# Sreyan88/audio-ssl

Hardware: AMD Instinct MI355X
Metric: upstream clips/sec (1s@16kHz, 64-mel) (higher is better)
Workload: dtype bf16; 1 GPU; delores-m upstream step (log-mel + 2 views + q/k conv encoders + MoCo + 3 Barlow heads + bwd + SGD), 1 s @ 16 kHz, 64 mel, batch 512/GPU, queue 65536; global_batch=512, parallelism=dp1

## Files before the change

audio-ssl_amd/csrc/bnpool.hip:

```cpp
#include "common.h"

namespace {

template <typename T_, bool SQ>
__global__ __launch_bounds__(256) void colstats_kernel(const T_* __restrict__ x, long M, int C, long ld, int rows_per_block,
                                                       double* __restrict__ sum, double* __restrict__ sumsq) {
    __shared__ float red[256][17];
    const int cg = threadIdx.x & 7, r0 = threadIdx.x >> 3;
    const int col0 = blockIdx.y * 64 + cg * 8;
    const long row_begin = (long)blockIdx.x * rows_per_block;
    const long row_end = min(M, row_begin + rows_per_block);
    x += (long)blockIdx.z * M * ld;
    sum += (long)blockIdx.z * C;
    if (SQ) sumsq += (long)blockIdx.z * C;
    float s[8], q[8];
#pragma unroll
    for (int i = 0; i < 8; ++i) { s[i] = 0.f; q[i] = 0.f; }
    if (col0 < C)
        for (long r = row_begin + r0; r < row_end; r += 32) {
            const Vec8<T_> v = Vec8<T_>::load(x + r * ld + col0);
#pragma unroll
            for (int i = 0; i < 8; ++i) { const float f = v.get(i); s[i] += f; if (SQ) q[i] += f * f; }
        }
#pragma unroll
// ... 369 lines not shown
    const int k8 = (int)(idx % 72);
    long pix = idx / 72;
    const int tap = k8 >> 3, c8 = k8 & 7;
    const int f = (int)(pix % Fi);
    const long r = pix / Fi;
    const int t = (int)(r % Ti);
    const long n = r / Ti;
    const int ff = f + tap / 3 - 1, tt = t + tap % 3 - 1;
    Vec8<T_> v = Vec8<T_>::zero();
    if (ff >= 0 && ff < Fi && tt >= 0 && tt < Ti) v = Vec8<T_>::load(X + (((n * Ti + tt) * Fi + ff) * 64 + c8 * 8));
    v.store(col + idx * 8);
}

template <typename T_>
__global__ void pack_conv_w_kernel(const float* __restrict__ W, T_* __restrict__ Wf, T_* __restrict__ Wd) {
    const int idx = blockIdx.x * 256 + threadIdx.x;
    if (idx >= 64 * 576) return;
    const int row = idx / 576, k = idx % 576, tap = k / 64, c = k % 64;
    Wf[idx] = from_f32<T_>(W[(row * 64 + c) * 9 + tap]);
    Wd[idx] = from_f32<T_>(W[(c * 64 + row) * 9 + (8 - tap)]);
}

template <typename T_>
__global__ void pack_conv_w2_kernel(const float* __restrict__ Wa, T_* __restrict__ Wfa, T_* __restrict__ Wda,
                                    const float* __restrict__ Wb, T_* __restrict__ Wfb, T_* __restrict__ Wdb) {
    const int idx = blockIdx.x * 256 + threadIdx.x;
    if (idx >= 64 * 576) return;
    const float* W = blockIdx.y ? Wb : Wa;
    T_* Wf = blockIdx.y ? Wfb : Wfa;
    T_* Wd = blockIdx.y ? Wdb : Wda;
    const int row = idx / 576, k = idx % 576, tap = k / 64, c = k % 64;
    Wf[idx] = from_f32<T_>(W[(row * 64 + c) * 9 + tap]);
    Wd[idx] = from_f32<T_>(W[(c * 64 + row) * 9 + (8 - tap)]);
}

__global__ void unpack_conv_dw_kernel(const float* __restrict__ dWp, float* __restrict__ dW) {
    const int idx = blockIdx.x * 256 + threadIdx.x;
    if (idx >= 64 * 576) return;
    const int co = idx / 576, k = idx % 576, tap = k / 64, ci = k % 64;
    dW[(co * 64 + ci) * 9 + tap] += dWp[idx];
}

}

#define DISPATCH_T(dtype, CALL_F32, CALL_BF16) do { if ((dtype) == 0) { CALL_F32; } else { CALL_BF16; } } while (0)

extern "C" int audiossl_colstats(int dtype, const void* x, int groups, long M, int C, long ld, int want_sq, double* sum,
                                 double* sumsq, void* stream) {
    ASSL_REQUIRE(x && sum && groups > 0 && M > 0 && C > 0 && (C % 8) == 0 && (ld % 8) == 0);
    ASSL_REQUIRE((dtype == 0 || dtype == 1) && (!want_sq || sumsq));
    hipStream_t s = static_cast<hipStream_t>(stream);
    const size_t nb = sizeof(double) * C * groups;
    if (want_sq && sumsq == sum + (size_t)C * groups) {
        ASSL_ZERO(sum, 2 * nb, s);
    } else {
        ASSL_ZERO(sum, nb, s);
        if (want_sq) ASSL_ZERO(sumsq, nb, s);
    }
    const int slabs = (C + 63) / 64;
    long it = (M * slabs * groups + 32L * 2048 - 1) / (32L * 2048);
    it = it < 1 ? 1 : (it > 128 ? 128 : it);
    const int rpb = 32 * (int)it;
    const dim3 grid(ceil_div(M, rpb), slabs, groups);
#define CS(TT, SQ) hipLaunchKernelGGL((colstats_kernel<TT, SQ>), grid, dim3(256), 0, s, static_cast<const TT*>(x), M, C, ld, rpb, sum, sumsq)
    if (dtype == 0) { if (want_sq) CS(float, true); else CS(float, false); }
    else            { if (want_sq) CS(bf16, true);  else CS(bf16, false); }
#undef CS
    ASSL_LAUNCH_CHECK();
}

extern "C" int audiossl_bn_finalize(const double* sum, const double* sumsq, int groups, double count, int C,
                                    const float* gamma, const float* beta, float* running_mean, float* running_var,
                                    float momentum, float eps, float* scale, float* shift, float* save_mean, float* save_rstd,
                                    void* stream) {
    ASSL_REQUIRE(sum && sumsq && scale && shift && save_mean && save_rstd && C > 0 && count > 0 && groups > 0);
    hipLaunchKernelGGL(bn_finalize_kernel, dim3(ceil_div(C, 256)), dim3(256), 0, static_cast<hipStream_t>(stream), sum, sumsq,
                       groups, count, C, gamma, beta, running_mean, running_var, momentum, eps, scale, shift, save_mean, save_rstd);
    ASSL_LAUNCH_CHECK();
}

extern "C" int audiossl_bn_relu_pool_fwd(int dtype, int ydtype, const void* Y, const float* scale, const float* shift, void* P,
                                         int N, int Ti, int Fi, void* stream) {
    ASSL_REQUIRE(Y && scale && shift && P && N > 0 && Ti >= 2 && Fi >= 2 && (Fi % 2) == 0 && (dtype == 0 || dtype == 1));
    ASSL_REQUIRE(ydtype == 0 || ydtype == dtype);
    const long total = (long)N * (Ti / 2) * (Fi / 2) * 8;
    hipStream_t s = static_cast<hipStream_t>(stream);
#define PF(TY, TO) hipLaunchKernelGGL((bn_relu_pool_fwd_kernel<TY, TO>), dim3(ceil_div(total, 256)), dim3(256), 0, s, \
        static_cast<const TY*>(Y), scale, shift, static_cast<TO*>(P), N, Ti, Fi)
    if (dtype == 0) PF(float, float); else if (ydtype == 0) PF(float, bf16); else PF(bf16, bf16);
#undef PF
    ASSL_LAUNCH_CHECK();
}

extern "C" int audiossl_bn_relu_pool_train_fwd(int dtype, int ydtype, const void* Y, const double* sum, const double* sumsq,
                                               int stat_replicas, double count,
                                               const float* gamma, const float* beta, float* running_mean, float* running_var,
                                               float momentum, float eps, void* P, float* scale, float* shift, float* save_mean,
                                               float* save_rstd, int N, int Ti, int Fi, void* stream) {
    ASSL_REQUIRE(Y && sum && sumsq && gamma && beta && P && scale && shift && save_mean && save_rstd && count > 0.0);
    ASSL_REQUIRE(stat_replicas >= 1 && (stat_replicas == 1 || sumsq == sum + 64));
    ASSL_REQUIRE(N > 0 && Ti >= 2 && Fi >= 2 && (Fi % 2) == 0 && (dtype == 0 || dtype == 1) && (ydtype == 0 || ydtype == dtype));
    const long total = (long)N * (Ti / 2) * (Fi / 2) * 8;
    hipStream_t s = static_cast<hipStream_t>(stream);
#define PF(TY, TO) hipLaunchKernelGGL((bn_relu_pool_train_fwd_kernel<TY, TO>), dim3(ceil_div(total, 256)), dim3(256), 0, s,          \
        static_cast<const TY*>(Y), sum, sumsq, stat_replicas, count, gamma, beta, running_mean, running_var, momentum, eps,      \
        static_cast<TO*>(P),                                                                                                      \
        scale, shift, save_mean, save_rstd, N, Ti, Fi)
    if (dtype == 0) PF(float, float); else if (ydtype == 0) PF(float, bf16); else PF(bf16, bf16);
#undef PF
    ASSL_LAUNCH_CHECK();
}

extern "C" int audiossl_tmean_fwd(int dtype, int out_f32, const void* P, void* xl, int N, int To, int Fo, void* stream) {
    ASSL_REQUIRE(P && xl && N > 0 && To > 0 && Fo > 0 && (dtype == 0 || dtype == 1));
    hipStream_t s = static_cast<hipStream_t>(stream);
#define TM(TI, TO_) hipLaunchKernelGGL((tmean_fwd_kernel<TI, TO_>), dim3(ceil_div(Fo * 8, 64), N), dim3(256), 0, s, \
        static_cast<const TI*>(P), static_cast<TO_*>(xl), N, To, Fo)
    if (dtype == 0) TM(float, float); else if (out_f32) TM(bf16, float); else TM(bf16, bf16);
#undef TM
    ASSL_LAUNCH_CHECK();
}

extern "C" int audiossl_tmean3_fwd(int dtype, int out_f32, const void* P1, void* x1, const float* x1_parts, int To1, int Fo1,
                                   const void* P2, void* x2, int To2, int Fo2, const void* P3, void* x3, int To3, int Fo3, int N,
                                   void* stream) {
    ASSL_REQUIRE(x1 && P2 && x2 && P3 && x3 && N > 0 && To1 > 0 && To2 > 0 && To3 > 0 && Fo1 > 0 && Fo2 > 0 && Fo3 > 0);
    ASSL_REQUIRE((P1 != nullptr) != (x1_parts != nullptr) && (!x1_parts || (out_f32 && dtype == 1)));
    ASSL_REQUIRE(dtype == 0 || dtype == 1);
    hipStream_t s = static_cast<hipStream_t>(stream);
    Tmean3 a{{P1, P2, P3}, {x1, x2, x3}, {To1, To2, To3}, {Fo1, Fo2, Fo3}, x1_parts};
    const int gx = ceil_div(max(Fo1, max(Fo2, Fo3)) * 8, 64);
#define TM3(TI, TO_) hipLaunchKernelGGL((tmean3_fwd_kernel<TI, TO_>), dim3(gx, N, 3), dim3(256), 0, s, a, N)
    if (dtype == 0) TM3(float, float); else if (out_f32) TM3(bf16, float); else TM3(bf16, bf16);
#undef TM3
    ASSL_LAUNCH_CHECK();
}

namespace {
__global__ void add_stat_kernel(const float* __restrict__ stat, float* dgamma, float* dbeta) {
    const int c = threadIdx.x;
    if (c < 64) { dbeta[c] += stat[c]; dgamma[c] += stat[64 + c]; }
}
}

static int bn_relu_pool_bwd_run(int phase, int dtype, int ydtype, int gdtype, const void* Y, const void* P, const void* dP, const void* dxl,
                                const float* scale, const float* shift, const float* mean, const float* rstd, float* stat,
                                const float* gstat, double count, void* dY, float* dgamma, float* dbeta, int N, int Ti, int Fi,
                                void* stream) {
    ASSL_REQUIRE(Y && dP && scale && shift && mean && rstd && stat);
    ASSL_REQUIRE(N > 0 && Ti >= 2 && Fi >= 2 && (Fi % 2) == 0 && (dtype == 0 || dtype == 1) && (gdtype == 0 || gdtype == dtype));
    ASSL_REQUIRE(ydtype == 0 || ydtype == dtype);
    ASSL_REQUIRE(phase == 1 || (dY && dgamma && dbeta));
    hipStream_t s = static_cast<hipStream_t>(stream);
    if (phase != 2) ASSL_ZERO(stat, sizeof(float) * 128 * 33, s);
    const long total = (long)N * ((Ti + 1) / 2) * (Fi / 2) * 8;
    const int grid = ceil_div(total, 256);
    const float inv_To = 1.f / (float)(Ti / 2);
    const float inv_count = (float)(1.0 / (phase == 2 ? count : (double)N * Ti * Fi));
    float* apply_stat = phase == 2 ? const_cast<float*>(gstat) : stat;
    const int fold = phase == 0;
#define BW(TY, AP, TG, TO, ST) hipLaunchKernelGGL((bn_relu_pool_bwd_kernel<TY, AP, TG, TO>), dim3(grid), dim3(256), 0, s,              \
        static_cast<const TY*>(Y), static_cast<const TG*>(dP), static_cast<const TG*>(dxl), inv_To, scale, shift, mean, rstd, ST, \
        inv_count, static_cast<TO*>(dY), N, Ti, Fi, (AP) ? fold : 0, dgamma, dbeta)
#define BWP(TG, TO) hipLaunchKernelGGL((bn_pool_bwd_stats_p_kernel<TO, TG>), dim3(pgrid), dim3(256), 0, s, static_cast<const TO*>(P),          \
        static_cast<const TG*>(dP), static_cast<const TG*>(dxl), inv_To, scale, shift, mean, rstd, stat, N, Ti / 2, Fi / 2)
#define BW2(TY, TG, TO) do { if (phase != 2) { if (P) BWP(TG, TO); else BW(TY, false, TG, TO, stat);                                       \
                                               if (!fold) hipLaunchKernelGGL(stat_reduce_kernel, dim3(1), dim3(128), 0, s, stat); }          \
                             if (phase != 1) BW(TY, true, TG, TO, apply_stat); } while (0)
    const long ptotal = (long)N * (Ti / 2) * (Fi / 2) * 8;
    const int pgrid = (int)min((long)2048, (ptotal + 255) / 256);
    if (dtype == 0) BW2(float, float, float);
    else if (ydtype == 0 && gdtype == 0) BW2(float, float, bf16);
    else if (ydtype == 0) BW2(float, bf16, bf16);
    else if (gdtype == 0) BW2(bf16, float, bf16);
    else BW2(bf16, bf16, bf16);
#undef BW2
#undef BWP
#undef BW
    if (phase == 2) hipLaunchKernelGGL(add_stat_kernel, dim3(1), dim3(64), 0, s, stat, dgamma, dbeta);
    ASSL_LAUNCH_CHECK();
}

extern "C" int audiossl_bn_relu_pool_bwd(int dtype, int ydtype, int gdtype, const void* Y, const void* dP, const void* dxl, const float* scale,
                                         const float* shift, const float* mean, const float* rstd, float* stat, void* dY,
                                         float* dgamma, float* dbeta, int N, int Ti, int Fi, void* stream) {
    return bn_relu_pool_bwd_run(0, dtype, ydtype, gdtype, Y, nullptr, dP, dxl, scale, shift, mean, rstd, stat, nullptr, 0.0, dY, dgamma, dbeta, N,
                                Ti, Fi, stream);
}
extern "C" int audiossl_bn_relu_pool_bwd_p(int dtype, int ydtype, int gdtype, const void* Y, const void* P, const void* dP, const void* dxl,
                                           const float* scale, const float* shift, const float* mean, const float* rstd, float* stat,
                                           void* dY, float* dgamma, float* dbeta, int N, int Ti, int Fi, void* stream) {
    ASSL_REQUIRE(P);
    return bn_relu_pool_bwd_run(0, dtype, ydtype, gdtype, Y, P, dP, dxl, scale, shift, mean, rstd, stat, nullptr, 0.0, dY, dgamma, dbeta, N,
                                Ti, Fi, stream);
}
extern "C" int audiossl_bn_relu_pool_bwd_stats(int dtype, int ydtype, int gdtype, const void* Y, const void* dP, const void* dxl,
                                               const float* scale, const float* shift, const float* mean, const float* rstd,
                                               float* stat, int N, int Ti, int Fi, void* stream) {
    return bn_relu_pool_bwd_run(1, dtype, ydtype, gdtype, Y, nullptr, dP, dxl, scale, shift, mean, rstd, stat, nullptr, 0.0, nullptr, nullptr,
                                nullptr, N, Ti, Fi, stream);
}
extern "C" int audiossl_bn_relu_pool_bwd_apply(int dtype, int ydtype, int gdtype, const void* Y, const void* dP, const void* dxl,
                                               const float* scale, const float* shift, const float* mean, const float* rstd,
                                               float* stat, const float* gstat, double count_global, void* dY, float* dgamma,
                                               float* dbeta, int N, int Ti, int Fi, void* stream) {
    ASSL_REQUIRE(gstat && count_global > 1.0);
    return bn_relu_pool_bwd_run(2, dtype, ydtype, gdtype, Y, nullptr, dP, dxl, scale, shift, mean, rstd, stat, gstat, count_global, dY, dgamma,
                                dbeta, N, Ti, Fi, stream);
}

extern "C" int audiossl_im2col3x3(int dtype, const void* X, void* col, int N, int Ti, int Fi, void* stream) {
    ASSL_REQUIRE(X && col && N > 0 && Ti > 0 && Fi > 0 && (dtype == 0 || dtype == 1));
    const long total = (long)N * Ti * Fi * 72;
    ASSL_REQUIRE((total + 255) / 256 < 2147483647L);
    hipStream_t s = static_cast<hipStream_t>(stream);
    DISPATCH_T(dtype,
        hipLaunchKernelGGL(im2col_kernel<float>, dim3(ceil_div(total, 256)), dim3(256), 0, s, static_cast<const float*>(X),
                           static_cast<float*>(col), N, Ti, Fi),
        hipLaunchKernelGGL(im2col_kernel<bf16>, dim3(ceil_div(total, 256)), dim3(256), 0, s, static_cast<const bf16*>(X),
                           static_cast<bf16*>(col), N, Ti, Fi));
    ASSL_LAUNCH_CHECK();
}

extern "C" int audiossl_pack_conv_w(int dtype, const float* W, void* Wf, void* Wd, void* stream) {
    ASSL_REQUIRE(W && Wf && Wd && (dtype == 0 || dtype == 1));
    hipStream_t s = static_cast<hipStream_t>(stream);
    DISPATCH_T(dtype,
        hipLaunchKernelGGL(pack_conv_w_kernel<float>, dim3(144), dim3(256), 0, s, W, static_cast<float*>(Wf), static_cast<float*>(Wd)),
        hipLaunchKernelGGL(pack_conv_w_kernel<bf16>, dim3(144), dim3(256), 0, s, W, static_cast<bf16*>(Wf), static_cast<bf16*>(Wd)));
    ASSL_LAUNCH_CHECK();
}

extern "C" int audiossl_pack_conv_w2(int dtype, const float* Wa, void* Wfa, void* Wda, const float* Wb, void* Wfb, void* Wdb, void* stream) {
    ASSL_REQUIRE(Wa && Wfa && Wda && Wb && Wfb && Wdb && (dtype == 0 || dtype == 1));
    hipStream_t s = static_cast<hipStream_t>(stream);
    DISPATCH_T(dtype,
        hipLaunchKernelGGL(pack_conv_w2_kernel<float>, dim3(144, 2), dim3(256), 0, s, Wa, static_cast<float*>(Wfa), static_cast<float*>(Wda),
                           Wb, static_cast<float*>(Wfb), static_cast<float*>(Wdb)),
        hipLaunchKernelGGL(pack_conv_w2_kernel<bf16>, dim3(144, 2), dim3(256), 0, s, Wa, static_cast<bf16*>(Wfa), static_cast<bf16*>(Wda),
                           Wb, static_cast<bf16*>(Wfb), static_cast<bf16*>(Wdb)));
    ASSL_LAUNCH_CHECK();
}

extern "C" int audiossl_unpack_conv_dw(const float* dWp, float* dW, void* stream) {
    ASSL_REQUIRE(dWp && dW);
    hipLaunchKernelGGL(unpack_conv_dw_kernel, dim3(144), dim3(256), 0, static_cast<hipStream_t>(stream), dWp, dW);
    ASSL_LAUNCH_CHECK();
}
```

audio-ssl_amd/csrc/conv.hip:

```cpp
#include <cstdlib>
#include "common.h"

namespace {

constexpr int CH = 64, KTOT = 576;
constexpr int WPITCH = KTOT + 8;
constexpr int PIXP = 72;
constexpr int PIXW = 96;

typedef __attribute__((address_space(3))) bf16x4* lds4_t;

struct ConvArgs {
    const bf16* X; const bf16* W; const float* bias; bf16* Y; double* sum; double* sumsq;
    int Ti, rows_total, tiles, out_f32, dbg, stat_rep;
};

template <int FI, int PITCH, int NTH = 256>
struct Halo {
    static constexpr int TT = 256 / FI;
    static constexpr int COLS = FI + 2;
    static constexpr int ELEMS = (TT + 2) * COLS * PITCH;
    static constexpr int NV = ((TT + 2) * FI * 8 + NTH - 1) / NTH;
    static constexpr int NVEC = (TT + 2) * FI * 8;
    Vec8<bf16> r[NV];
// ... 11 lines not shown
        for (int i = 0; i < NV; ++i) {
            const int v = threadIdx.x + i * NTH;
            const int row = v / (FI * 8), rem = v % (FI * 8);
            if (v < NVEC) r[i].store(lds + (row * COLS + (rem >> 3) + 1) * PITCH + (rem & 7) * 8);
        }
    }
    __device__ __forceinline__ static void zero_border(bf16* lds) {
        for (int i = threadIdx.x; i < (TT + 2) * 2 * 8; i += NTH) {
            const int row = i / 16, side = (i >> 3) & 1, c8 = i & 7;
            Vec8<bf16>::zero().store(lds + (row * COLS + side * (FI + 1)) * PITCH + c8 * 8);
        }
    }
};

template <int FI, int NW>
__global__ __launch_bounds__(64 * NW, 1) void conv3x3_kernel(ConvArgs a) {
    using H = Halo<FI, PIXP, 64 * NW>;
    constexpr int RT = 8 / NW;
    constexpr int TT = H::TT, COLS = H::COLS;
    extern __shared__ __attribute__((aligned(16))) char smem[];
    bf16* const wl = reinterpret_cast<bf16*>(smem);
    bf16* const hl = wl + CH * WPITCH;
    float* const red = reinterpret_cast<float*>(hl);

    const int lane = threadIdx.x & 63, wave = threadIdx.x >> 6;
    const int m = lane & 31, h = lane >> 5;
    for (int v = threadIdx.x; v < CH * KTOT / 8; v += 64 * NW) {
        const int row = v / (KTOT / 8), c = v % (KTOT / 8);
        Vec8<bf16>::load(a.W + row * KTOT + c * 8).store(wl + row * WPITCH + c * 8);
    }
    H::zero_border(hl);

    float ssum[2][16], ssq[2][16];
#pragma unroll
    for (int j = 0; j < 2; ++j)
#pragma unroll
        for (int r = 0; r < 16; ++r) { ssum[j][r] = 0.f; ssq[j][r] = 0.f; }
    f32x4 bias4[2][4];
#pragma unroll
    for (int j = 0; j < 2; ++j)
#pragma unroll
        for (int q = 0; q < 4; ++q)
            bias4[j][q] = a.bias ? *reinterpret_cast<const f32x4*>(a.bias + j * 32 + 8 * q + 4 * h) : f32x4{0.f, 0.f, 0.f, 0.f};
    H halo;
    int tile = blockIdx.x;
    if (tile < a.tiles) { halo.load(a.X, tile * TT, a.rows_total); halo.put(hl); }
    __syncthreads();

    for (; tile < a.tiles; tile += gridDim.x) {
        const int g0 = tile * TT;
        const int next = tile + gridDim.x;
        if (next < a.tiles && !(a.dbg & 2)) halo.load(a.X, next * TT, a.rows_total);

        int tl[RT], fcol[RT];
        bool ok[RT][3];
#pragma unroll
        for (int i = 0; i < RT; ++i) {
            const int rt = RT * wave + i;
            tl[i] = FI == 32 ? rt : 2 * rt + (m >> 4);
            fcol[i] = FI == 32 ? m : (m & 15);
            const int g = g0 + tl[i];
            const int ti = g % a.Ti;
#pragma unroll
            for (int dt = 0; dt < 3; ++dt) ok[i][dt] = g < a.rows_total && ti + dt - 1 >= 0 && ti + dt - 1 < a.Ti;
        }
        f32x16 acc[RT][2];
#pragma unroll
        for (int i = 0; i < RT; ++i)
#pragma unroll
            for (int j = 0; j < 2; ++j)
#pragma unroll
                for (int r = 0; r < 16; ++r) acc[i][j][r] = 0.f;

        if (!(a.dbg & 4))
#pragma unroll
        for (int tap = 0; tap < 9; ++tap) {
            const int dt = tap % 3, df = tap / 3;
#pragma unroll
            for (int cc = 0; cc < 4; ++cc) {
                Vec8<bf16> fa[RT], fb[2];
#pragma unroll
                for (int i = 0; i < RT; ++i) {
                    const bf16* p = hl + ((tl[i] + dt) * COLS + fcol[i] + df) * PIXP + cc * 16 + 8 * h;
                    fa[i] = ok[i][dt] ? Vec8<bf16>::load(p) : Vec8<bf16>::zero();
                }
#pragma unroll
                for (int j = 0; j < 2; ++j) fb[j] = Vec8<bf16>::load(wl + (j * 32 + m) * WPITCH + tap * 64 + cc * 16 + 8 * h);
#pragma unroll
                for (int i = 0; i < RT; ++i)
#pragma unroll
                    for (int j = 0; j < 2; ++j)
                        acc[i][j] = __builtin_amdgcn_mfma_f32_32x32x16_bf16(fb[j].v, fa[i].v, acc[i][j], 0, 0, 0);
            }
        }
#pragma unroll
        for (int i = 0; i < RT; ++i) {
            const int g = g0 + tl[i];
            if (g < a.rows_total && !(a.dbg & 1)) {
                const long o = ((long)g * FI + fcol[i]) * CH;
#pragma unroll
                for (int j = 0; j < 2; ++j)
#pragma unroll
                    for (int q = 0; q < 4; ++q) {
                        f32x4 v;
#pragma unroll
                        for (int e = 0; e < 4; ++e) {
                            v[e] = acc[i][j][4 * q + e] + bias4[j][q][e];
                            ssum[j][4 * q + e] += v[e];
                            ssq[j][4 * q + e] += v[e] * v[e];
                        }
                        const int co = j * 32 + 8 * q + 4 * h;
                        if (a.out_f32) *reinterpret_cast<f32x4*>(reinterpret_cast<float*>(a.Y) + o + co) = v;
                        else *reinterpret_cast<bf16x4*>(a.Y + o + co) = bf16x4{(bf16)v[0], (bf16)v[1], (bf16)v[2], (bf16)v[3]};
                    }
            }
        }
        __syncthreads();
        if (next < a.tiles) halo.put(hl);
        __syncthreads();
    }
    if (a.sum) {
#pragma unroll
        for (int j = 0; j < 2; ++j)
#pragma unroll
            for (int r = 0; r < 16; ++r) {
                float s = ssum[j][r], q = ssq[j][r];
#pragma unroll
                for (int o = 16; o > 0; o >>= 1) { s += __shfl_xor(s, o, 64); q += __shfl_xor(q, o, 64); }
                if (m == 0) {
                    const int co = j * 32 + (r & 3) + 8 * (r >> 2) + 4 * h;
                    red[(wave * 64 + co) * 2] = s; red[(wave * 64 + co) * 2 + 1] = q;
                }
            }
        __syncthreads();
        if (threadIdx.x < 128) {
            const int c = threadIdx.x >> 1, k = threadIdx.x & 1;
            double t = 0.0;
#pragma unroll
            for (int w = 0; w < NW; ++w) t += (double)red[(w * 64 + c) * 2 + k];
            const int rep = (blockIdx.x % a.stat_rep) * 128;
            atomicAdd(k == 0 ? &a.sum[rep + c] : &a.sumsq[rep + c], t);
        }
    }
}

template <int FI>
struct WsGeom {
    static constexpr int TT = 256 / FI, COLS = FI + 2, ROWS = TT + 2, SEGS = FI / 8;
    static constexpr int UNITS = ROWS * SEGS;
    static constexpr int UPW = (UNITS + 3) / 4;
    static constexpr int BYTES = ROWS * COLS * 128;
};

template <int FI, bool STATS, bool F32OUT, int PF = 2>
__global__ __launch_bounds__(256, 1) void conv3x3_ws_kernel(ConvArgs a) {
    using G = WsGeom<FI>;
    constexpr int TT = G::TT, COLS = G::COLS;
    typedef __attribute__((address_space(3))) void* lptr_t;
    extern __shared__ __attribute__((aligned(16))) char smem[];
    float* const biasl = reinterpret_cast<float*>(smem + 2 * G::BYTES);
    float* const red = biasl + 64;
    constexpr int OPIX = F32OUT ? 256 : 128;
    char* const stg = reinterpret_cast<char*>(red + 4 * 64 * 2) + (threadIdx.x >> 6) * 64 * OPIX;
    char* const zblk = reinterpret_cast<char*>(red + 4 * 64 * 2) + 4 * 64 * OPIX;
    if (threadIdx.x < 32) *reinterpret_cast<f32x4*>(zblk + threadIdx.x * 16) = f32x4{0.f, 0.f, 0.f, 0.f};

    const int lane = threadIdx.x & 63, wave = __builtin_amdgcn_readfirstlane(threadIdx.x >> 6);
    const int m = lane & 31, h = lane >> 5;
    long* const rts = (!STATS && (a.dbg & 16) && threadIdx.x == 0 && (blockIdx.x == 0 || blockIdx.x == gridDim.x - 1))
                          ? reinterpret_cast<long*>(a.sum) + 64 + (blockIdx.x ? 8 : 0) : nullptr;
    if (rts) rts[0] = __builtin_amdgcn_s_memrealtime();

    {
        bf16* const wl = reinterpret_cast<bf16*>(smem);
        Vec8<bf16> tmp[CH * KTOT / 8 / 256];
#pragma unroll
        for (int k = 0; k < CH * KTOT / 8 / 256; ++k) tmp[k] = Vec8<bf16>::load(a.W + (threadIdx.x + 256 * k) * 8);
#pragma unroll
        for (int k = 0; k < CH * KTOT / 8 / 256; ++k) {
            const int v = threadIdx.x + 256 * k, row = v / (KTOT / 8), c = v % (KTOT / 8);
            tmp[k].store(wl + row * WPITCH + c * 8);
        }
        __syncthreads();
    }
    Vec8<bf16> wr[2][36];
#pragma unroll
    for (int j = 0; j < 2; ++j)
#pragma unroll
        for (int ks = 0; ks < 36; ++ks)
            wr[j][ks] = Vec8<bf16>::load(reinterpret_cast<const bf16*>(smem) + (j * 32 + m) * WPITCH + ks * 16 + 8 * h);
#pragma unroll
    for (int ks = 0; ks < 36; ++ks) {
        asm volatile("" : "+v"(wr[0][ks].v));
        asm volatile("" : "+a"(wr[1][ks].v));
    }

    __syncthreads();
    for (int i = threadIdx.x; i < 2 * G::ROWS * 2 * 8; i += 256) {
        const int b = i / (G::ROWS * 16), r = (i / 16) % G::ROWS, side = (i >> 3) & 1, c8 = i & 7;
        *reinterpret_cast<f32x4*>(smem + b * G::BYTES + (r * COLS + side * (FI + 1)) * 128 + c8 * 16) = f32x4{0.f, 0.f, 0.f, 0.f};
    }
    if (threadIdx.x < 64) biasl[threadIdx.x] = a.bias ? a.bias[threadIdx.x] : 0.f;

    if (rts) { asm volatile("s_waitcnt vmcnt(0)" ::: "memory"); rts[3] = __builtin_amdgcn_s_memrealtime(); }
    const __amdgpu_buffer_rsrc_t rsrc = __builtin_amdgcn_make_buffer_rsrc(const_cast<bf16*>(a.X), 0, (unsigned)((long)a.rows_total * FI * 128), 0x00020000);
    const int pl = lane >> 3, cp = lane & 7;
    const int key0 = ((1 + pl) >> 1) & 7;
    const int voff0 = pl * 128 + ((cp ^ key0) << 4), voff1 = pl * 128 + ((cp ^ key0 ^ 4) << 4);
    auto dma_unit = [&](int g0, char* buf, int i) {
        {
            const int u = wave + 4 * i;
            if (u < G::UNITS) {
                const int row = u / G::SEGS, seg = u % G::SEGS;
                const int gr = g0 - 1 + row;
                const int so = (gr >= 0 && gr < a.rows_total) ? (gr * FI + 8 * seg) * 128 : 0x7FFFFF00;
                __builtin_amdgcn_raw_ptr_buffer_load_lds(rsrc, (lptr_t)(buf + (row * COLS + 1 + 8 * seg) * 128), 16, (seg & 1) ? voff1 : voff0, so, 0, 0);
            }
        }
    };
    auto dma_tile = [&](int g0, char* buf) {
#pragma unroll
        for (int i = 0; i < G::UPW; ++i) dma_unit(g0, buf, i);
    };

    int tl[2];
    const int fcol = FI == 32 ? m : (m & 15);
#pragma unroll
    for (int i = 0; i < 2; ++i) {
        const int rt = 2 * wave + i;
        tl[i] = FI == 32 ? rt : 2 * rt + (m >> 4);
    }
    int hs[3];
#pragma unroll
    for (int df = 0; df < 3; ++df) hs[df] = (h ^ (((fcol + df) >> 1) & 7)) << 4;

    constexpr int NS = F32OUT ? 4 : 8;
    float ssum[NS], ssq[NS];
    if (STATS) {
#pragma unroll
        for (int e = 0; e < NS; ++e) { ssum[e] = 0.f; ssq[e] = 0.f; }
    }

    int tile = blockIdx.x, cur = 0;
    if (tile < a.tiles) dma_tile(tile * TT, smem);
    asm volatile("s_waitcnt vmcnt(0) lgkmcnt(0)" ::: "memory");
    __builtin_amdgcn_s_barrier();

    long* const ts = (!STATS && (a.dbg & 16) && blockIdx.x == 0 && threadIdx.x == 0) ? reinterpret_cast<long*>(a.sum) : nullptr;
    int tsi = 0;
    if (rts) rts[1] = __builtin_amdgcn_s_memrealtime();
    for (; tile < a.tiles; tile += gridDim.x, cur ^= 1) {
        if (ts) ts[tsi++] = __builtin_amdgcn_s_memtime();
        const int g0 = tile * TT;
        const int next = tile + gridDim.x;
        if (next < a.tiles && !(a.dbg & 2)) dma_tile(next * TT, smem + (cur ^ 1) * G::BYTES);
        const char* const hl = smem + cur * G::BYTES;

        int bdt[2][3];
#pragma unroll
        for (int i = 0; i < 2; ++i) {
            const int g = g0 + tl[i];
            const int ti = g % a.Ti;
#pragma unroll
            for (int dt = 0; dt < 3; ++dt) {
                const bool ok = g < a.rows_total && ti + dt - 1 >= 0 && ti + dt - 1 < a.Ti;
                bdt[i][dt] = ok ? (int)(size_t)((lptr_t)const_cast<char*>(hl)) + ((tl[i] + dt) * COLS + fcol) * 128
                                : (int)(size_t)((lptr_t)zblk);
            }
        }
        f32x16 acc[2][2];
#pragma unroll
        for (int j = 0; j < 2; ++j)
#pragma unroll
            for (int q = 0; q < 4; ++q) {
                const f32x4 b4 = *reinterpret_cast<const f32x4*>(biasl + j * 32 + 8 * q + 4 * h);
#pragma unroll
                for (int e = 0; e < 4; ++e) { acc[0][j][4 * q + e] = b4[e]; acc[1][j][4 * q + e] = b4[e]; }
            }

        Vec8<bf16> fa[PF + 1][2];
        auto fetch = [&](int ks, Vec8<bf16> (&f)[2]) {
            const int tap = ks >> 2, cc = ks & 3, dt = tap % 3, df = tap / 3;
#pragma unroll
            for (int i = 0; i < 2; ++i)
                f[i] = Vec8<bf16>::load(reinterpret_cast<const bf16*>((const char*)(lptr_t)(size_t)(bdt[i][dt] + df * 128 + (hs[df] ^ (cc * 32)))));
        };
        if (!(a.dbg & 4)) {
#pragma unroll
        for (int ks = 0; ks < PF; ++ks) fetch(ks, fa[ks]);
#pragma unroll
        for (int ks = 0; ks < 36; ++ks) {
            if (ks + PF < 36) fetch(ks + PF, fa[(ks + PF) % (PF + 1)]);
            __builtin_amdgcn_sched_barrier(0);
            Vec8<bf16> (&f)[2] = fa[ks % (PF + 1)];
#pragma unroll
            for (int i = 0; i < 2; ++i) {
#pragma unroll
                for (int j = 0; j < 2; ++j)
                    acc[i][j] = __builtin_amdgcn_mfma_f32_32x32x16_bf16(wr[j][ks].v, f[i].v, acc[i][j], 0, 0, 0);
            }
            __builtin_amdgcn_sched_barrier(0);
        }
        }
        if (ts) ts[tsi++] = __builtin_amdgcn_s_memtime();
        asm volatile("s_waitcnt vmcnt(0)" ::: "memory");
        if (ts) ts[tsi++] = __builtin_amdgcn_s_memtime();
        if (!(a.dbg & 1)) {
#pragma unroll
            for (int i = 0; i < 2; ++i) {
                char* const st = stg + i * 32 * OPIX;
#pragma unroll
                for (int j = 0; j < 2; ++j)
#pragma unroll
                    for (int q = 0; q < 4; ++q) {
                        const int slot = j * 8 + 2 * q + h;
                        const f32x4 v = f32x4{acc[i][j][4 * q], acc[i][j][4 * q + 1], acc[i][j][4 * q + 2], acc[i][j][4 * q + 3]};
                        if (F32OUT) *reinterpret_cast<f32x4*>(st + m * 256 + ((slot ^ (m & 15)) << 4)) = v;
                        else *reinterpret_cast<bf16x4*>(st + m * 128 + ((slot ^ ((m >> 1) & 15)) << 3)) =
                                 bf16x4{(bf16)v[0], (bf16)v[1], (bf16)v[2], (bf16)v[3]};
                    }
            }
            asm volatile("s_waitcnt lgkmcnt(0)" ::: "memory");
#pragma unroll
            for (int i = 0; i < 2; ++i) {
                const char* const st = stg + i * 32 * OPIX;
                const int grow = g0 + (2 * wave + i) * (32 / FI);
                const int prow_ok = a.rows_total - grow;
                char* const yrow = reinterpret_cast<char*>(a.Y) + (long)grow * FI * 64 * (F32OUT ? 4 : 2);
                if (F32OUT) {
#pragma unroll
                    for (int it = 0; it < 8; ++it) {
                        const int p = it * 4 + (lane >> 4), c = lane & 15;
                        const f32x4 v = *reinterpret_cast<const f32x4*>(st + p * 256 + ((c ^ (p & 15)) << 4));
                        if ((p >> (FI == 32 ? 5 : 4)) < prow_ok) {
                            *reinterpret_cast<f32x4*>(yrow + p * 256 + c * 16) = v;
                            if (STATS) {
#pragma unroll
                                for (int e = 0; e < 4; ++e) { ssum[e] += v[e]; ssq[e] += v[e] * v[e]; }
                            }
                        }
                    }
                } else {
#pragma unroll
                    for (int it = 0; it < 4; ++it) {
                        const int p = it * 8 + (lane >> 3), c = lane & 7, k = (p >> 1) & 15;
                        f32x4 v = *reinterpret_cast<const f32x4*>(st + p * 128 + ((c ^ (k >> 1)) << 4));
                        if (k & 1) v = f32x4{v[2], v[3], v[0], v[1]};
                        if ((p >> (FI == 32 ? 5 : 4)) < prow_ok) {
                            *reinterpret_cast<f32x4*>(yrow + p * 128 + c * 16) = v;
                            if (STATS) {
                                const bf16x8 hv = __builtin_bit_cast(bf16x8, v);
#pragma unroll
                                for (int e = 0; e < 8; ++e) {
                                    const float x = (float)hv[e];
                                    ssum[e] += x; ssq[e] += x * x;
                                }
                            }
                        }
                    }
                }
            }
        }
        if (ts) ts[tsi++] = __builtin_amdgcn_s_memtime();
        asm volatile("s_waitcnt lgkmcnt(0)" ::: "memory");
        __builtin_amdgcn_s_barrier();
    }
    if (rts) rts[2] = __builtin_amdgcn_s_memrealtime();
    if (STATS) {
#pragma unroll
        for (int e = 0; e < NS; ++e) {
            float s = ssum[e], q = ssq[e];
#pragma unroll
            for (int o = 64 / NS; o < 64; o <<= 1) { s += __shfl_xor(s, o, 64); q += __shfl_xor(q, o, 64); }
            if (lane < 64 / NS) {
                const int co = lane * NS + e;
                red[(wave * 64 + co) * 2] = s; red[(wave * 64 + co) * 2 + 1] = q;
            }
        }
        __syncthreads();
        if (threadIdx.x < 128) {
            const int c = threadIdx.x >> 1, k = threadIdx.x & 1;
            double t = 0.0;
#pragma unroll
            for (int w = 0; w < 4; ++w) t += (double)red[(w * 64 + c) * 2 + k];
            const int rep = (blockIdx.x % a.stat_rep) * 128;
            atomicAdd(k == 0 ? &a.sum[rep + c] : &a.sumsq[rep + c], t);
        }
    }
}

__host__ __device__ __forceinline__ int wg_cot(int w, int n) { return n < 8 ? (n & 1) : (w & 1); }
__host__ __device__ __forceinline__ int wg_nt(int w, int n) { return n < 8 ? 4 * w + (n >> 1) : 16 + (w >> 1); }

struct WgradArgs {
    const bf16* dY; const bf16* X; float* dW; int Ti, rows_total, tiles;
    float* partial;
    int dbg;
};

template <int FI, int KG>
__global__ __launch_bounds__(256 * KG, 1) void conv3x3_wgrad_kernel(WgradArgs a) {
    using H = Halo<FI, PIXW, 256 * KG>;
    constexpr int TT = H::TT, COLS = H::COLS;
    constexpr int NTH = 256 * KG;
    constexpr int NVY = 256 * 8 / NTH;
    extern __shared__ __attribute__((aligned(16))) char smem[];
    bf16* const yl = reinterpret_cast<bf16*>(smem);
    bf16* const hl = yl + 256 * PIXW;

    const int lane = threadIdx.x & 63, wave = (threadIdx.x >> 6) & 3, grp = threadIdx.x >> 8;
    const int h = lane >> 5, half = (lane >> 4) & 1, q = (lane & 15) >> 2, p = lane & 3;
    H::zero_border(hl);

    f32x16 acc[9];
#pragma unroll
    for (int n = 0; n < 9; ++n)
#pragma unroll
        for (int r = 0; r < 16; ++r) acc[n][r] = 0.f;

    H halo;
    Vec8<bf16> ry[NVY];
    auto load_y = [&](int g0) {
#pragma unroll
        for (int i = 0; i < NVY; ++i) {
            const int v = threadIdx.x + i * NTH;
            const long pix = (long)g0 * FI + (v >> 3);
            ry[i] = pix < (long)a.rows_total * FI ? Vec8<bf16>::load(a.dY + pix * CH + (v & 7) * 8) : Vec8<bf16>::zero();
        }
    };
    auto put_y = [&]() {
#pragma unroll
        for (int i = 0; i < NVY; ++i) {
            const int v = threadIdx.x + i * NTH;
            ry[i].store(yl + (v >> 3) * PIXW + (v & 7) * 8);
        }
    };
    int tile = blockIdx.x;
    if (tile < a.tiles) { halo.load(a.X, tile * TT, a.rows_total); load_y(tile * TT); halo.put(hl); put_y(); }
    __syncthreads();

    for (; tile < a.tiles; tile += gridDim.x) {
        const int g0 = tile * TT;
        const int next = tile + gridDim.x;
        if (next < a.tiles && !(a.dbg & 2)) { halo.load(a.X, next * TT, a.rows_total); load_y(next * TT); }

#pragma unroll 1
        for (int ks = grp * (16 / KG); ks < (grp + 1) * (16 / KG) && !(a.dbg & 4); ++ks) {
            const int t_local = FI == 32 ? (ks >> 1) : ks;
            const int f0 = FI == 32 ? (ks & 1) * 16 : 0;
            const int g = g0 + t_local;
            if (g >= a.rows_total) break;
            const int ti = g % a.Ti;
            const bool okt[3] = {ti - 1 >= 0, true, ti + 1 < a.Ti};
            bf16x8 fa[2];
#pragma unroll
            for (int c2 = 0; c2 < 2; ++c2) {
                const bf16* ay = yl + (ks * 16 + 8 * h + q) * PIXW + c2 * 32 + 16 * half + 4 * p;
                const bf16x4 a0 = __builtin_amdgcn_ds_read_tr16_b64_v4bf16((lds4_t)ay);
                const bf16x4 a1 = __builtin_amdgcn_ds_read_tr16_b64_v4bf16((lds4_t)(ay + 4 * PIXW));
                fa[c2] = bf16x8{a0[0], a0[1], a0[2], a0[3], a1[0], a1[1], a1[2], a1[3]};
            }
            bf16x8 fb;
#pragma unroll
            for (int n = 0; n < 9; ++n) {
                if (n == 8 || (n & 1) == 0) {
                    const int nt = wg_nt(wave, n), tap = nt >> 1, cih = nt & 1;
                    const int dt = tap % 3, df = tap / 3;
                    const bf16* bx = hl + ((t_local + dt) * COLS + f0 + df + 8 * h + q) * PIXW + cih * 32 + 16 * half + 4 * p;
                    const bf16x4 b0 = __builtin_amdgcn_ds_read_tr16_b64_v4bf16((lds4_t)bx);
                    const bf16x4 b1 = __builtin_amdgcn_ds_read_tr16_b64_v4bf16((lds4_t)(bx + 4 * PIXW));
                    const bf16 z = (bf16)0.f;
                    fb = okt[dt] ? bf16x8{b0[0], b0[1], b0[2], b0[3], b1[0], b1[1], b1[2], b1[3]} : bf16x8{z, z, z, z, z, z, z, z};
                }
                const int c2 = wg_cot(wave, n);
                acc[n] = __builtin_amdgcn_mfma_f32_32x32x16_bf16(c2 ? fa[1] : fa[0], fb, acc[n], 0, 0, 0);
            }
        }
        __syncthreads();
        if (next < a.tiles) { halo.put(hl); put_y(); }
        __syncthreads();
    }
    if (a.partial) {
        if (KG == 2) {
            f32x4* xch = reinterpret_cast<f32x4*>(smem);
            __syncthreads();
            if (grp == 1) {
#pragma unroll
                for (int n = 0; n < 9; ++n)
#pragma unroll
                    for (int r4 = 0; r4 < 4; ++r4)
                        xch[((wave * 9 + n) * 4 + r4) * 64 + lane] = f32x4{acc[n][4 * r4], acc[n][4 * r4 + 1], acc[n][4 * r4 + 2], acc[n][4 * r4 + 3]};
            }
            __syncthreads();
            if (grp == 1) return;
            f32x4* part = reinterpret_cast<f32x4*>(a.partial + (long)blockIdx.x * (CH * KTOT));
#pragma unroll
            for (int n = 0; n < 9; ++n)
#pragma unroll
                for (int r4 = 0; r4 < 4; ++r4) {
                    const f32x4 o = xch[((wave * 9 + n) * 4 + r4) * 64 + lane];
                    part[((wave * 9 + n) * 4 + r4) * 64 + lane] = f32x4{acc[n][4 * r4] + o[0], acc[n][4 * r4 + 1] + o[1], acc[n][4 * r4 + 2] + o[2], acc[n][4 * r4 + 3] + o[3]};
                }
            return;
        }
        f32x4* part = reinterpret_cast<f32x4*>(a.partial + (long)blockIdx.x * (CH * KTOT));
#pragma unroll
        for (int n = 0; n < 9; ++n)
#pragma unroll
            for (int r4 = 0; r4 < 4; ++r4)
                part[((wave * 9 + n) * 4 + r4) * 64 + lane] = f32x4{acc[n][4 * r4], acc[n][4 * r4 + 1], acc[n][4 * r4 + 2], acc[n][4 * r4 + 3]};
        return;
    }
#pragma unroll
    for (int n = 0; n < 9; ++n) {
        const int nt = wg_nt(wave, n), tap = nt >> 1, cih = nt & 1;
        const int col = tap * 64 + cih * 32 + (lane & 31);
#pragma unroll
        for (int r = 0; r < 16; ++r) {
            const int co = wg_cot(wave, n) * 32 + (r & 3) + 8 * (r >> 2) + 4 * h;
            atomicAdd(&a.dW[co * KTOT + col], acc[n][r]);
        }
    }
}

__global__ __launch_bounds__(256) void wgrad_reduce_kernel(const float* __restrict__ partial, int nparts, float* __restrict__ dW) {
    const int i = blockIdx.x * 256 + threadIdx.x;
    if (i >= CH * KTOT) return;
    float s0 = 0.f, s1 = 0.f, s2 = 0.f, s3 = 0.f;
    int w = blockIdx.y;
    const int step = gridDim.y;
    for (; w + 3 * step < nparts; w += 4 * step) {
        s0 += partial[(long)w * (CH * KTOT) + i];
        s1 += partial[(long)(w + step) * (CH * KTOT) + i];
        s2 += partial[(long)(w + 2 * step) * (CH * KTOT) + i];
        s3 += partial[(long)(w + 3 * step) * (CH * KTOT) + i];
    }
    for (; w < nparts; w += step) s0 += partial[(long)w * (CH * KTOT) + i];
    const int e = i & 3, lane = (i >> 2) & 63, r4 = (i >> 8) & 3, wn = i >> 10;
    const int wave = wn / 9, n = wn - wave * 9;
    const int nt = wg_nt(wave, n), tap = nt >> 1, cih = nt & 1;
    const int col = tap * 64 + cih * 32 + (lane & 31);
    const int co = wg_cot(wave, n) * 32 + e + 8 * r4 + 4 * (lane >> 5);
    atomicAdd(&dW[co * KTOT + col], (s0 + s1) + (s2 + s3));
}

template <typename K>
int set_lds(K kernel, size_t bytes) {
    return hipFuncSetAttribute(reinterpret_cast<const void*>(kernel), hipFuncAttributeMaxDynamicSharedMemorySize, (int)bytes) ==
           hipSuccess ? 0 : -1;
}

}

extern "C" int audiossl_conv3x3_fwd(const void* X, const void* W, const float* bias, void* Y, int out_f32, double* sum,
                                    double* sumsq, int stat_replicas, int N, int Ti, int Fi, void* stream) {
    ASSL_REQUIRE(X && W && Y && N > 0 && Ti > 0 && (Fi == 32 || Fi == 16) && (!sum == !sumsq));
    ASSL_REQUIRE(stat_replicas >= 1 && stat_replicas <= 64 && (stat_replicas == 1 || !sum || sumsq == sum + 64));
    if (!ASSL_ALIGNED16(X) || !ASSL_ALIGNED16(W) || !ASSL_ALIGNED16(Y)) return ASSL_EALIGN;
    hipStream_t s = static_cast<hipStream_t>(stream);
#ifdef AUDIOSSL_ABLATE
    static const int conv_dbg = getenv("AUDIOSSL_CONV_DBG") ? atoi(getenv("AUDIOSSL_CONV_DBG")) : 0;
#else
    constexpr int conv_dbg = 0;
#endif
    if (sum && !(conv_dbg & 16)) {
        if (sumsq == sum + 64) {
            ASSL_ZERO(sum, sizeof(double) * 128 * stat_replicas, s);
        } else {
            ASSL_ZERO(sum, sizeof(double) * 64, s);
            ASSL_ZERO(sumsq, sizeof(double) * 64, s);
        }
    }
    const int rows = N * Ti, TT = 256 / Fi, tiles = (rows + TT - 1) / TT;
    ConvArgs a{static_cast<const bf16*>(X), static_cast<const bf16*>(W), bias, static_cast<bf16*>(Y), sum, sumsq, Ti, rows, tiles, out_f32, conv_dbg, stat_replicas};
    const int grid = tiles < 256 ? tiles : 256;
    static const int ws = getenv("AUDIOSSL_CONV_WS") ? atoi(getenv("AUDIOSSL_CONV_WS")) : 1;
    if (ws && (long)rows * Fi * 128 < 0x7FFFFF00L) {
        static bool wattr[8] = {false, false, false, false, false, false, false, false};
#define WS_LAUNCH(FI_, ST_, F32_, SLOT)                                                                    \
    do {                                                                                                  \
        const size_t lds = 2 * WsGeom<FI_>::BYTES + sizeof(float) * (64 + 4 * 64 * 2) + 4 * 64 * (F32_ ? 256 : 128) + 512; \
        if (!wattr[SLOT]) { if (set_lds(conv3x3_ws_kernel<FI_, ST_, F32_>, lds)) return ASSL_ELAUNCH; wattr[SLOT] = true; } \
        hipLaunchKernelGGL((conv3x3_ws_kernel<FI_, ST_, F32_>), dim3(grid), dim3(256), lds, s, a);       \
    } while (0)
        if (Fi == 32) {
            if (sum && !(conv_dbg & 16)) { if (out_f32) WS_LAUNCH(32, true, true, 0); else WS_LAUNCH(32, true, false, 1); }
            else     { if (out_f32) WS_LAUNCH(32, false, true, 2); else WS_LAUNCH(32, false, false, 3); }
        } else {
            if (sum) { if (out_f32) WS_LAUNCH(16, true, true, 4); else WS_LAUNCH(16, true, false, 5); }
            else     { if (out_f32) WS_LAUNCH(16, false, true, 6); else WS_LAUNCH(16, false, false, 7); }
        }
#undef WS_LAUNCH
        ASSL_LAUNCH_CHECK();
    }
    static const int nw = getenv("AUDIOSSL_CONV_WAVES") ? atoi(getenv("AUDIOSSL_CONV_WAVES")) : 8;
    static bool attr[4] = {false, false, false, false};
#define CONV_LAUNCH(FI_, NW_, SLOT)                                                                       \
    do {                                                                                                  \
        const size_t lds = sizeof(bf16) * (CH * WPITCH + Halo<FI_, PIXP>::ELEMS);                         \
        if (!attr[SLOT]) { if (set_lds(conv3x3_kernel<FI_, NW_>, lds)) return ASSL_ELAUNCH; attr[SLOT] = true; } \
        hipLaunchKernelGGL((conv3x3_kernel<FI_, NW_>), dim3(grid), dim3(64 * NW_), lds, s, a);           \
    } while (0)
    if (Fi == 32) { if (nw == 8) CONV_LAUNCH(32, 8, 0); else CONV_LAUNCH(32, 4, 1); }
    else          { if (nw == 8) CONV_LAUNCH(16, 8, 2); else CONV_LAUNCH(16, 4, 3); }
#undef CONV_LAUNCH
    ASSL_LAUNCH_CHECK();
}

extern "C" int audiossl_conv3x3_wgrad(const void* dY, const void* X, float* dWp, float* workspace, long workspace_floats, int N,
                                      int Ti, int Fi, void* stream) {
    ASSL_REQUIRE(dY && X && dWp && N > 0 && Ti > 0 && (Fi == 32 || Fi == 16));
    if (!ASSL_ALIGNED16(X) || !ASSL_ALIGNED16(dY)) return ASSL_EALIGN;
    hipStream_t s = static_cast<hipStream_t>(stream);
    const int rows = N * Ti, TT = 256 / Fi, tiles = (rows + TT - 1) / TT;
    const int grid = tiles < 256 ? tiles : 256;
    const bool two_stage = workspace != nullptr && workspace_floats >= (long)grid * CH * KTOT;
#ifdef AUDIOSSL_ABLATE
    static const int wg_dbg = getenv("AUDIOSSL_CONV_DBG") ? atoi(getenv("AUDIOSSL_CONV_DBG")) : 0;
#else
    constexpr int wg_dbg = 0;
#endif
    WgradArgs a{static_cast<const bf16*>(dY), static_cast<const bf16*>(X), dWp, Ti, rows, tiles, two_stage ? workspace : nullptr, wg_dbg};
    static const int kg_env = getenv("AUDIOSSL_WGRAD_KG") ? atoi(getenv("AUDIOSSL_WGRAD_KG")) : 0;
    const int kg = kg_env ? kg_env : (two_stage ? 2 : 1);
    static bool attr[4] = {false, false, false, false};
#define WGRAD_LAUNCH(FI_, KG_, SLOT)                                                                      \
    do {                                                                                                  \
        const size_t lds = max(sizeof(bf16) * (256 * PIXW + Halo<FI_, PIXW>::ELEMS), (size_t)(KG_ == 2 ? 4 * 9 * 16 * 64 * 4 : 0)); \
        if (!attr[SLOT]) { if (set_lds(conv3x3_wgrad_kernel<FI_, KG_>, lds)) return ASSL_ELAUNCH; attr[SLOT] = true; } \
        hipLaunchKernelGGL((conv3x3_wgrad_kernel<FI_, KG_>), dim3(grid), dim3(256 * KG_), lds, s, a);    \
    } while (0)
    if (Fi == 32) { if (kg == 2) WGRAD_LAUNCH(32, 2, 0); else WGRAD_LAUNCH(32, 1, 1); }
    else          { if (kg == 2) WGRAD_LAUNCH(16, 2, 2); else WGRAD_LAUNCH(16, 1, 3); }
#undef WGRAD_LAUNCH
    if (two_stage)
        hipLaunchKernelGGL(wgrad_reduce_kernel, dim3(CH * KTOT / 256, 8), dim3(256), 0, s, workspace, grid, dWp);
    ASSL_LAUNCH_CHECK();
}
```

audio-ssl_amd/csrc/heads.hip:

```cpp
#include "common.h"

namespace {

template <typename T_, typename TO>
__global__ __launch_bounds__(256) void maxmean_fwd_kernel(const T_* __restrict__ H, TO* __restrict__ y, uint8_t* __restrict__ arg,
                                                          int N, int Tt, int D) {
    const long idx = (long)blockIdx.x * 256 + threadIdx.x;
    const int D8 = D / 8;
    if (idx >= (long)N * D8) return;
    const int d8 = (int)(idx % D8);
    const long n = idx / D8;
    float mx[8], sm[8];
    int am[8];
    for (int t = 0; t < Tt; ++t) {
        const Vec8<T_> v = Vec8<T_>::load(H + ((n * Tt + t) * D + d8 * 8));
#pragma unroll
        for (int i = 0; i < 8; ++i) {
            const float f = v.get(i);
            if (t == 0) { mx[i] = f; sm[i] = f; am[i] = 0; }
            else { sm[i] += f; if (f > mx[i]) { mx[i] = f; am[i] = t; } }
        }
    }
    Vec8<TO> o;
    const float inv = 1.f / (float)Tt;
#pragma unroll
    for (int i = 0; i < 8; ++i) { o.set(i, mx[i] + sm[i] * inv); arg[n * D + d8 * 8 + i] = (uint8_t)am[i]; }
    o.store(y + n * D + d8 * 8);
}

template <typename T_, typename TG>
__global__ __launch_bounds__(256) void maxmean_bwd_kernel(const TG* __restrict__ dy, const uint8_t* __restrict__ arg,
                                                          const T_* __restrict__ H, T_* __restrict__ dA, int N, int Tt, int D) {
    const long idx = (long)blockIdx.x * 256 + threadIdx.x;
    const int D8 = D / 8;
    if (idx >= (long)N * Tt * D8) return;
    const int d8 = (int)(idx % D8);
    const long r = idx / D8;
    const int t = (int)(r % Tt);
    const long n = r / Tt;
    const Vec8<TG> g = Vec8<TG>::load(dy + n * D + d8 * 8);
    const Vec8<T_> h = Vec8<T_>::load(H + idx * 8);
    Vec8<T_> o;
    const float inv = 1.f / (float)Tt;
#pragma unroll
    for (int i = 0; i < 8; ++i) {
        const float gi = g.get(i);
        const float v = gi * inv + (arg[n * D + d8 * 8 + i] == t ? gi : 0.f);
        o.set(i, h.get(i) > 0.f ? v : 0.f);
    }
    o.store(dA + idx * 8);
}

template <typename TA, typename T_>
__global__ __launch_bounds__(256) void colbn_fwd_kernel(const TA* __restrict__ a, const float* __restrict__ scale,
                                                        const float* __restrict__ shift, int relu, T_* __restrict__ h, long M, int C,
                                                        int groups) {
    const long idx = (long)blockIdx.x * 256 + threadIdx.x;
    const int C8 = C / 8;
    if (idx >= (long)groups * M * C8) return;
    const int c8 = (int)(idx % C8);
    const int grp = (int)(idx / (M * C8));
    scale += (long)grp * C;
    shift += (long)grp * C;
    const Vec8<TA> v = Vec8<TA>::load(a + idx * 8);
    Vec8<T_> o;
#pragma unroll
    for (int i = 0; i < 8; ++i) {
        float f = scale[c8 * 8 + i] * v.get(i) + shift[c8 * 8 + i];
        o.set(i, relu ? fmaxf(f, 0.f) : f);
    }
    o.store(h + idx * 8);
}

template <typename TA, typename TG>
__global__ __launch_bounds__(256) void colbn_bwd_stats_kernel(const TA* __restrict__ a, const TG* __restrict__ dh,
                                                              const float* __restrict__ scale, const float* __restrict__ shift,
                                                              const float* __restrict__ mean, const float* __restrict__ rstd,
                                                              int relu, long M, int C, int rows_per_block,
                                                              double* __restrict__ sg, double* __restrict__ sgx) {
    __shared__ float red[256][17];
    const int cg = threadIdx.x & 7, r0 = threadIdx.x >> 3;
    const int col0 = blockIdx.y * 64 + cg * 8;
    const long rb = (long)blockIdx.x * rows_per_block, re = min(M, rb + rows_per_block);
    {
        const long go = (long)blockIdx.z * C, ro = (long)blockIdx.z * M * C;
        a += ro; dh += ro; scale += go; shift += go; mean += go; rstd += go; sg += go; sgx += go;
    }
    float s[8], q[8], sc[8], sh[8], mu[8], rs[8];
#pragma unroll
    for (int i = 0; i < 8; ++i) {
        s[i] = 0.f; q[i] = 0.f;
        sc[i] = scale[col0 + i]; sh[i] = shift[col0 + i]; mu[i] = mean[col0 + i]; rs[i] = rstd[col0 + i];
    }
    for (long r = rb + r0; r < re; r += 32) {
        const Vec8<TA> va = Vec8<TA>::load(a + r * C + col0);
        const Vec8<TG> vg = Vec8<TG>::load(dh + r * C + col0);
#pragma unroll
        for (int i = 0; i < 8; ++i) {
            const float x = va.get(i);
            float g = vg.get(i);
            if (relu && !(sc[i] * x + sh[i] > 0.f)) g = 0.f;
            s[i] += g;
            q[i] += g * (x - mu[i]) * rs[i];
        }
    }
#pragma unroll
    for (int i = 0; i < 8; ++i) { red[threadIdx.x][i] = s[i]; red[threadIdx.x][8 + i] = q[i]; }
    __syncthreads();
    if (threadIdx.x < 128) {
        const int g = threadIdx.x >> 4, k = threadIdx.x & 15;
        double t = 0.0;
        for (int r = 0; r < 32; ++r) t += (double)red[r * 8 + g][k];
        const int c = blockIdx.y * 64 + g * 8 + (k & 7);
        if (k < 8) atomicAdd(&sg[c], t); else atomicAdd(&sgx[c], t);
    }
}

template <typename TA, typename TG, typename T_>
__global__ __launch_bounds__(256) void colbn_bwd_apply_kernel(const TA* __restrict__ a, const TG* __restrict__ dh,
                                                              const float* __restrict__ scale, const float* __restrict__ shift,
                                                              const float* __restrict__ mean, const float* __restrict__ rstd,
                                                              int relu, long M, int C, int groups, const double* __restrict__ sg,
                                                              const double* __restrict__ sgx, T_* __restrict__ da,
                                                              float* dgamma, float* dbeta, float invM) {
    const long idx = (long)blockIdx.x * 256 + threadIdx.x;
    const int C8 = C / 8;
    if (idx >= (long)groups * M * C8) return;
    const int c8 = (int)(idx % C8);
    const long grow = idx / C8;
    const int grp = (int)(grow / M);
    const long row = grow - (long)grp * M;
    {
        const long go = (long)grp * C;
        scale += go; shift += go; mean += go; rstd += go; sg += go; sgx += go;
    }
    const Vec8<TA> va = Vec8<TA>::load(a + idx * 8);
    const Vec8<TG> vg = Vec8<TG>::load(dh + idx * 8);
    const Vec8<float> vsc = Vec8<float>::load(scale + c8 * 8), vsh = Vec8<float>::load(shift + c8 * 8);
    const Vec8<float> vmu = Vec8<float>::load(mean + c8 * 8), vrs = Vec8<float>::load(rstd + c8 * 8);
    double dsg[8], dsx[8];
#pragma unroll
    for (int i = 0; i < 8; i += 2) {
        const double2 p = *reinterpret_cast<const double2*>(sg + c8 * 8 + i), q = *reinterpret_cast<const double2*>(sgx + c8 * 8 + i);
        dsg[i] = p.x; dsg[i + 1] = p.y; dsx[i] = q.x; dsx[i + 1] = q.y;
    }
    Vec8<T_> o;
#pragma unroll
    for (int i = 0; i < 8; ++i) {
        const int c = c8 * 8 + i;
        const float x = va.get(i);
        float g = vg.get(i);
        if (relu && !(vsc.get(i) * x + vsh.get(i) > 0.f)) g = 0.f;
        const float xhat = (x - vmu.get(i)) * vrs.get(i);
        const float mg = (float)dsg[i] * invM, mgx = (float)dsx[i] * invM;
        o.set(i, vsc.get(i) * (g - mg - xhat * mgx));
        if (row == 0 && dgamma) { atomicAdd(&dgamma[c], (float)sgx[c]); atomicAdd(&dbeta[c], (float)sg[c]); }
    }
    o.store(da + idx * 8);
}

template <int NS>
__device__ __forceinline__ void strip_reduce(const float (&part)[NS][8], float (*red)[65], double* tot) {
    const int cl = threadIdx.x & 3, r0 = threadIdx.x >> 2;
#pragma unroll
    for (int k = 0; k < NS; ++k) {
        __syncthreads();
#pragma unroll
        for (int i = 0; i < 8; ++i) red[r0][cl * 8 + i] = part[k][i];
        __syncthreads();
        if (threadIdx.x < 32) {
            double t = 0.0;
            for (int r = 0; r < 64; ++r) t += (double)red[r][threadIdx.x];
            tot[k * 32 + threadIdx.x] = t;
        }
    }
    __syncthreads();
}

template <typename TA, typename T_, int NR>
__device__ __forceinline__ void colbn_train_fwd_body(const TA* __restrict__ a, const float* __restrict__ gamma,
                                                              const float* __restrict__ beta, float* running_mean,
                                                              float* running_var, float momentum, float eps, int relu, int groups,
                                                              int M, int C, T_* __restrict__ h, float* __restrict__ scale,
                                                              float* __restrict__ shift, float* __restrict__ save_mean,
                                                              float* __restrict__ save_rstd) {
    __shared__ float red[64][65];
    __shared__ double tot[64];
    __shared__ float sc_s[32], sh_s[32];
    const int cl = threadIdx.x & 3, r0 = threadIdx.x >> 2;
    const int col0 = blockIdx.x * 32 + cl * 8;
    const int c = blockIdx.x * 32 + threadIdx.x;
    float rm = 0.f, rv = 0.f;
    if (threadIdx.x < 32 && running_mean) { rm = running_mean[c]; rv = running_var[c]; }
    Vec8<TA> vn[NR];
    auto fetch = [&](int g, Vec8<TA> (&dst)[NR]) {
        const TA* ag = a + (long)g * M * C;
#pragma unroll
        for (int j = 0; j < NR; ++j) {
            const int r = r0 + 64 * j;
            if (r < M) dst[j] = Vec8<TA>::load(ag + (long)r * C + col0);
        }
    };
    fetch(0, vn);
// ... 373 lines not shown
            f32x4 bv = first ? f32x4{0, 0, 0, 0} : *reinterpret_cast<f32x4*>(buf + i);
#pragma unroll
            for (int k = 0; k < 4; ++k) {
                float pk = pv[k], bk = bv[k];
                sgd_step(pk, gv[k], bk, lr, mom, wd, gscale, first);
                pv[k] = pk; bv[k] = bk;
            }
            *reinterpret_cast<f32x4*>(buf + i) = bv;
            *reinterpret_cast<f32x4*>(p + i) = pv;
            if (shadow) *reinterpret_cast<bf16x4*>(shadow + i) = bf16x4{(bf16)pv[0], (bf16)pv[1], (bf16)pv[2], (bf16)pv[3]};
            if (zero_grad) *reinterpret_cast<f32x4*>(g + i) = f32x4{0.f, 0.f, 0.f, 0.f};
        } else {
            for (long j = i; j < n; ++j) {
                float pj = p[j], b = first ? 0.f : buf[j];
                sgd_step(pj, g[j], b, lr, mom, wd, gscale, first);
                buf[j] = b;
                p[j] = pj;
                if (shadow) shadow[j] = (bf16)pj;
                if (zero_grad) g[j] = 0.f;
            }
        }
    }
}

__global__ __launch_bounds__(256) void sgd_segments_kernel(float* __restrict__ p, float* __restrict__ g, float* __restrict__ buf,
                                                           const long* __restrict__ segs, float lr, float mom, float wd, int first,
                                                           float gscale_host, const float* __restrict__ gscale_dev,
                                                           bf16* __restrict__ shadow, int zero_grad) {
    const float gscale = gscale_dev ? gscale_host * gscale_dev[0] : gscale_host;
    const long off = segs[2 * blockIdx.y], n = segs[2 * blockIdx.y + 1];
    for (long i = ((long)blockIdx.x * 256 + threadIdx.x) * 4; i < n; i += (long)gridDim.x * 1024) {
        const long e = off + i;
        if (i + 4 <= n) {
            f32x4 pv = *reinterpret_cast<f32x4*>(p + e);
            const f32x4 gv = *reinterpret_cast<const f32x4*>(g + e);
            f32x4 bv = first ? f32x4{0, 0, 0, 0} : *reinterpret_cast<f32x4*>(buf + e);
#pragma unroll
            for (int k = 0; k < 4; ++k) {
                float pk = pv[k], bk = bv[k];
                sgd_step(pk, gv[k], bk, lr, mom, wd, gscale, first);
                pv[k] = pk; bv[k] = bk;
            }
            *reinterpret_cast<f32x4*>(buf + e) = bv;
            *reinterpret_cast<f32x4*>(p + e) = pv;
            if (shadow) *reinterpret_cast<bf16x4*>(shadow + e) = bf16x4{(bf16)pv[0], (bf16)pv[1], (bf16)pv[2], (bf16)pv[3]};
            if (zero_grad) *reinterpret_cast<f32x4*>(g + e) = f32x4{0.f, 0.f, 0.f, 0.f};
        } else {
            for (long j = e; j < off + n; ++j) {
                float pj = p[j], b = first ? 0.f : buf[j];
                sgd_step(pj, g[j], b, lr, mom, wd, gscale, first);
                buf[j] = b;
                p[j] = pj;
                if (shadow) shadow[j] = (bf16)pj;
                if (zero_grad) g[j] = 0.f;
            }
        }
    }
}

__global__ __launch_bounds__(256) void zero_segments_kernel(float* __restrict__ g, const long* __restrict__ segs) {
    const long off = segs[2 * blockIdx.y], n = segs[2 * blockIdx.y + 1];
    for (long i = (long)blockIdx.x * 256 + threadIdx.x; i < n; i += (long)gridDim.x * 256) g[off + i] = 0.f;
}

__global__ __launch_bounds__(256) void ema_kernel(float* __restrict__ pk, const float* __restrict__ pq, long n, float m,
                                                  bf16* __restrict__ shadow) {
    const float om = 1.f - m;
    const bool vec = ((reinterpret_cast<size_t>(pk) | reinterpret_cast<size_t>(pq)) & 15) == 0 && (reinterpret_cast<size_t>(shadow) & 7) == 0;
    const long n4 = vec ? n / 4 : 0;
    for (long i = (long)blockIdx.x * 256 + threadIdx.x; i < n4; i += (long)gridDim.x * 256) {
        f32x4 a = *reinterpret_cast<const f32x4*>(pk + i * 4);
        const f32x4 b = *reinterpret_cast<const f32x4*>(pq + i * 4);
#pragma unroll
        for (int k = 0; k < 4; ++k) a[k] = a[k] * m + b[k] * om;
        *reinterpret_cast<f32x4*>(pk + i * 4) = a;
        if (shadow) *reinterpret_cast<bf16x4*>(shadow + i * 4) = bf16x4{(bf16)a[0], (bf16)a[1], (bf16)a[2], (bf16)a[3]};
    }
    for (long i = n4 * 4 + (long)blockIdx.x * 256 + threadIdx.x; i < n; i += (long)gridDim.x * 256) {
        const float v = pk[i] * m + pq[i] * om;
        pk[i] = v;
        if (shadow) shadow[i] = (bf16)v;
    }
}

template <typename T_>
__global__ __launch_bounds__(256) void cast_kernel(const float* __restrict__ src, T_* __restrict__ dst, long n, int vec) {
    const long n8 = vec ? n / 8 : 0;
    for (long i = (long)blockIdx.x * 256 + threadIdx.x; i < n8; i += (long)gridDim.x * 256) {
        const Vec8<float> v = Vec8<float>::load(src + i * 8);
        Vec8<T_> o;
#pragma unroll
        for (int k = 0; k < 8; ++k) o.set(k, v.get(k));
        o.store(dst + i * 8);
    }
    for (long i = n8 * 8 + (long)blockIdx.x * 256 + threadIdx.x; i < n; i += (long)gridDim.x * 256) dst[i] = from_f32<T_>(src[i]);
}

template <typename T_>
__global__ __launch_bounds__(256) void cast_back_kernel(const T_* __restrict__ src, float* __restrict__ dst, long n) {
    for (long i = (long)blockIdx.x * 256 + threadIdx.x; i < n; i += (long)gridDim.x * 256) dst[i] = to_f32(src[i]);
}

__global__ __launch_bounds__(256) void dropout_mask_kernel(uint8_t* __restrict__ keep, long n, unsigned long long seed, float p,
                                                           const long long* __restrict__ counter) {
    seed = dropout_seed(seed, counter);
    const unsigned int thr = dropout_threshold(p);
    auto bit = [&](long i) -> unsigned int { return dropout_keep(seed, i, thr); };
    const long n16 = ((reinterpret_cast<size_t>(keep) & 15) == 0) ? n / 16 : 0;
    for (long v = (long)blockIdx.x * 256 + threadIdx.x; v < n16; v += (long)gridDim.x * 256) {
        unsigned int w[4];
#pragma unroll
        for (int q = 0; q < 4; ++q) {
            const long i = v * 16 + q * 4;
            w[q] = bit(i) | (bit(i + 1) << 8) | (bit(i + 2) << 16) | (bit(i + 3) << 24);
        }
        *reinterpret_cast<uint4*>(keep + v * 16) = make_uint4(w[0], w[1], w[2], w[3]);
    }
    for (long i = n16 * 16 + (long)blockIdx.x * 256 + threadIdx.x; i < n; i += (long)gridDim.x * 256) keep[i] = (uint8_t)bit(i);
}

}

int g_assl_prezeroed = 0;
extern "C" int audiossl_set_prezeroed(int on) { g_assl_prezeroed = on ? 1 : 0; return ASSL_OK; }
const char* g_assl_last_kernel = "";
extern "C" int audiossl_last_kernel(char* name, int capacity) {
    ASSL_REQUIRE(name && capacity > 0);
    int i = 0;
    for (; g_assl_last_kernel[i] && i < capacity - 1; ++i) name[i] = g_assl_last_kernel[i];
    name[i] = 0;
    return ASSL_OK;
}

#define S_(stream) static_cast<hipStream_t>(stream)
#define GRID1(n) dim3((unsigned)(((long)(n) + 255) / 256))

extern "C" int audiossl_maxmean_fwd(int dtype, int out_f32, const void* H, void* y, uint8_t* arg, int N, int Tt, int D, void* stream) {
    ASSL_REQUIRE(H && y && arg && N > 0 && Tt > 0 && Tt < 256 && D > 0 && (D % 8) == 0 && (dtype == 0 || dtype == 1));
    const long total = (long)N * D / 8;
    if (dtype == 0) hipLaunchKernelGGL((maxmean_fwd_kernel<float, float>), GRID1(total), dim3(256), 0, S_(stream), (const float*)H, (float*)y, arg, N, Tt, D);
    else if (out_f32) hipLaunchKernelGGL((maxmean_fwd_kernel<bf16, float>), GRID1(total), dim3(256), 0, S_(stream), (const bf16*)H, (float*)y, arg, N, Tt, D);
    else            hipLaunchKernelGGL((maxmean_fwd_kernel<bf16, bf16>), GRID1(total), dim3(256), 0, S_(stream), (const bf16*)H, (bf16*)y, arg, N, Tt, D);
    ASSL_LAUNCH_CHECK();
}

extern "C" int audiossl_maxmean_bwd(int dtype, int gdtype, const void* dy, const uint8_t* arg, const void* H, void* dA, int N, int Tt,
                                    int D, void* stream) {
    ASSL_REQUIRE(dy && arg && H && dA && N > 0 && Tt > 0 && D > 0 && (D % 8) == 0 && (dtype == 0 || dtype == 1));
    ASSL_REQUIRE(gdtype == 0 || gdtype == dtype);
    const long total = (long)N * Tt * D / 8;
    if (dtype == 0) hipLaunchKernelGGL((maxmean_bwd_kernel<float, float>), GRID1(total), dim3(256), 0, S_(stream), (const float*)dy, arg, (const float*)H, (float*)dA, N, Tt, D);
    else if (gdtype == 0) hipLaunchKernelGGL((maxmean_bwd_kernel<bf16, float>), GRID1(total), dim3(256), 0, S_(stream), (const float*)dy, arg, (const bf16*)H, (bf16*)dA, N, Tt, D);
    else            hipLaunchKernelGGL((maxmean_bwd_kernel<bf16, bf16>), GRID1(total), dim3(256), 0, S_(stream), (const bf16*)dy, arg, (const bf16*)H, (bf16*)dA, N, Tt, D);
    ASSL_LAUNCH_CHECK();
}

extern "C" int audiossl_colbn_fwd(int dtype, int adtype, const void* a, const float* scale, const float* shift, int relu, void* h,
                                  int groups, long M, int C, void* stream) {
    ASSL_REQUIRE(a && scale && shift && h && groups > 0 && M > 0 && C > 0 && (C % 8) == 0 && (dtype == 0 || dtype == 1));
    ASSL_REQUIRE(adtype == 0 || adtype == dtype);
    const long total = groups * M * C / 8;
    if (dtype == 0) hipLaunchKernelGGL((colbn_fwd_kernel<float, float>), GRID1(total), dim3(256), 0, S_(stream), (const float*)a, scale, shift, relu, (float*)h, M, C, groups);
    else if (adtype == 0) hipLaunchKernelGGL((colbn_fwd_kernel<float, bf16>), GRID1(total), dim3(256), 0, S_(stream), (const float*)a, scale, shift, relu, (bf16*)h, M, C, groups);
    else hipLaunchKernelGGL((colbn_fwd_kernel<bf16, bf16>), GRID1(total), dim3(256), 0, S_(stream), (const bf16*)a, scale, shift, relu, (bf16*)h, M, C, groups);
    ASSL_LAUNCH_CHECK();
}

extern "C" int audiossl_colbn_train_fwd(int dtype, int adtype, const void* a, const float* gamma, const float* beta,
                                        float* running_mean, float* running_var, float momentum, float eps, int relu,
                                        int groups, long M, int C, void* h, float* scale, float* shift, float* save_mean,
                                        float* save_rstd, void* stream) {
    ASSL_REQUIRE(a && h && scale && shift && save_mean && save_rstd && groups > 0 && M > 0 && M <= 1024 && C > 0 && (C % 32) == 0);
    ASSL_REQUIRE((dtype == 0 || dtype == 1) && (adtype == 0 || adtype == dtype));
    ASSL_REQUIRE((running_mean == nullptr) == (running_var == nullptr));
    hipStream_t s = S_(stream);
#define TF(TA, TO) do {                                                                                                        \
    if (M <= 512) hipLaunchKernelGGL((colbn_train_fwd_kernel<TA, TO, 8>), dim3(C / 32), dim3(256), 0, s, (const TA*)a, gamma, beta, \
                                     running_mean, running_var, momentum, eps, relu, groups, (int)M, C, (TO*)h, scale, shift,    \
                                     save_mean, save_rstd);                                                                     \
    else hipLaunchKernelGGL((colbn_train_fwd_kernel<TA, TO, 16>), dim3(C / 32), dim3(256), 0, s, (const TA*)a, gamma, beta,      \
                            running_mean, running_var, momentum, eps, relu, groups, (int)M, C, (TO*)h, scale, shift, save_mean,  \
                            save_rstd); } while (0)
    if (dtype == 0) TF(float, float);
    else if (adtype == 0) TF(float, bf16);
    else TF(bf16, bf16);
#undef TF
    ASSL_LAUNCH_CHECK();
}

extern "C" int audiossl_colbn_bwd(int dtype, int adtype, int gdtype, const void* a, const void* dh, const float* scale,
                                  const float* shift, const float* mean, const float* rstd, int relu, int groups, long M, int C,
                                  double* tmp, void* da, float* dgamma, float* dbeta, void* stream) {
    ASSL_REQUIRE(a && dh && scale && shift && mean && rstd && tmp && da && groups > 0 && M > 0 && C > 0 && (C % 8) == 0);
    ASSL_REQUIRE((dtype == 0 || dtype == 1) && (C % 64) == 0 && (gdtype == 0 || gdtype == dtype) && (adtype == 0 || adtype == dtype));
    hipStream_t s = S_(stream);
    static const bool fused_ok = getenv("AUDIOSSL_BN_FUSED") ? atoi(getenv("AUDIOSSL_BN_FUSED")) != 0 : true;
    if (fused_ok && M <= 1024 && (C % 32) == 0) {
        dim3 fgrid(C / 32, groups);
#define CF(TA, TG, TO) do {                                                                                                    \
    if (M <= 512) hipLaunchKernelGGL((colbn_bwd_fused_kernel<TA, TG, TO, 8>), fgrid, dim3(256), 0, s, (const TA*)a, (const TG*)dh, \
                                     scale, shift, mean, rstd, relu, (int)M, C, (TO*)da, dgamma, dbeta);                        \
    else hipLaunchKernelGGL((colbn_bwd_fused_kernel<TA, TG, TO, 16>), fgrid, dim3(256), 0, s, (const TA*)a, (const TG*)dh,      \
                            scale, shift, mean, rstd, relu, (int)M, C, (TO*)da, dgamma, dbeta); } while (0)
        if (dtype == 0) CF(float, float, float);
        else if (adtype == 0 && gdtype == 0) CF(float, float, bf16);
        else if (adtype == 0) CF(float, bf16, bf16);
        else if (gdtype == 0) CF(bf16, float, bf16);
        else CF(bf16, bf16, bf16);
#undef CF
        ASSL_LAUNCH_CHECK();
    }
    ASSL_ZERO(tmp, sizeof(double) * 2 * C * groups, s);
    const int rpb = M >= 4096 ? 256 : 64;
    dim3 grid(ceil_div(M, rpb), C / 64, groups);
    const long total = groups * M * C / 8;
    const long GC = (long)groups * C;
#define CB(TA, TG, TO) do {                                                                                                           \
    hipLaunchKernelGGL((colbn_bwd_stats_kernel<TA, TG>), grid, dim3(256), 0, s, (const TA*)a, (const TG*)dh, scale, shift, mean, rstd,  \
                       relu, M, C, rpb, tmp, tmp + GC);                                                                               \
    hipLaunchKernelGGL((colbn_bwd_apply_kernel<TA, TG, TO>), GRID1(total), dim3(256), 0, s, (const TA*)a, (const TG*)dh, scale, shift,  \
                       mean, rstd, relu, M, C, groups, tmp, tmp + GC, (TO*)da, dgamma, dbeta, 1.f / (float)M); } while (0)
    if (dtype == 0) CB(float, float, float);
    else if (adtype == 0 && gdtype == 0) CB(float, float, bf16);
    else if (adtype == 0) CB(float, bf16, bf16);
    else if (gdtype == 0) CB(bf16, float, bf16);
    else CB(bf16, bf16, bf16);
#undef CB
    ASSL_LAUNCH_CHECK();
}

extern "C" int audiossl_colbn_bwd_stats(int dtype, int adtype, int gdtype, const void* a, const void* dh, const float* scale,
                                        const float* shift, const float* mean, const float* rstd, int relu, int groups, long M, int C,
                                        double* tmp, void* stream) {
    ASSL_REQUIRE(a && dh && scale && shift && mean && rstd && tmp && groups > 0 && M > 0 && C > 0 && (C % 64) == 0);
    ASSL_REQUIRE((dtype == 0 || dtype == 1) && (gdtype == 0 || gdtype == dtype) && (adtype == 0 || adtype == dtype));
    hipStream_t s = S_(stream);
    ASSL_ZERO(tmp, sizeof(double) * 2 * C * groups, s);
    const int rpb = M >= 4096 ? 256 : 64;
    dim3 grid(ceil_div(M, rpb), C / 64, groups);
    const long GC = (long)groups * C;
#define CS(TA, TG) hipLaunchKernelGGL((colbn_bwd_stats_kernel<TA, TG>), grid, dim3(256), 0, s, (const TA*)a, (const TG*)dh, scale, shift, \
                                      mean, rstd, relu, M, C, rpb, tmp, tmp + GC)
    if (dtype == 0 || (adtype == 0 && gdtype == 0)) CS(float, float);
    else if (adtype == 0) CS(float, bf16);
    else if (gdtype == 0) CS(bf16, float);
    else CS(bf16, bf16);
#undef CS
    ASSL_LAUNCH_CHECK();
}
extern "C" int audiossl_colbn_bwd_apply(int dtype, int adtype, int gdtype, const void* a, const void* dh, const float* scale,
                                        const float* shift, const float* mean, const float* rstd, int relu, int groups, long M, int C,
                                        const double* sums, double count, void* da, void* stream) {
    ASSL_REQUIRE(a && dh && scale && shift && mean && rstd && sums && da && groups > 0 && M > 0 && C > 0 && (C % 64) == 0 && count > 1.0);
    ASSL_REQUIRE((dtype == 0 || dtype == 1) && (gdtype == 0 || gdtype == dtype) && (adtype == 0 || adtype == dtype));
    hipStream_t s = S_(stream);
    const long total = groups * M * C / 8;
    const long GC = (long)groups * C;
    const float inv = (float)(1.0 / count);
#define CA(TA, TG, TO) hipLaunchKernelGGL((colbn_bwd_apply_kernel<TA, TG, TO>), GRID1(total), dim3(256), 0, s, (const TA*)a, (const TG*)dh, \
                                          scale, shift, mean, rstd, relu, M, C, groups, sums, sums + GC, (TO*)da, (float*)nullptr,          \
                                          (float*)nullptr, inv)
    if (dtype == 0) CA(float, float, float);
    else if (adtype == 0 && gdtype == 0) CA(float, float, bf16);
    else if (adtype == 0) CA(float, bf16, bf16);
    else if (gdtype == 0) CA(bf16, float, bf16);
    else CA(bf16, bf16, bf16);
#undef CA
    ASSL_LAUNCH_CHECK();
}

extern "C" int audiossl_colbn_train_fwd_multi(int count, int adtype, const void* const* a, const float* const* gamma,
                                              const float* const* beta, float* const* running_mean, float* const* running_var,
                                              float momentum, float eps, int relu, int groups, long M, int C, void* const* h,
                                              float* const* stats, void* stream) {
    ASSL_REQUIRE(count >= 1 && count <= MAXP && a && h && stats && groups > 0 && M > 0 && M <= 1024 && C > 0 && (C % 32) == 0);
    ASSL_REQUIRE(adtype == 0 || adtype == 1);
    BnFwdMulti m{};
    for (int p = 0; p < count; ++p) {
        ASSL_REQUIRE(a[p] && h[p] && stats[p]);
        m.a[p] = a[p]; m.h[p] = h[p]; m.st[p] = stats[p];
        m.gamma[p] = gamma ? gamma[p] : nullptr; m.beta[p] = beta ? beta[p] : nullptr;
        m.rm[p] = running_mean ? running_mean[p] : nullptr; m.rv[p] = running_var ? running_var[p] : nullptr;
        ASSL_REQUIRE((m.rm[p] == nullptr) == (m.rv[p] == nullptr));
    }
    hipStream_t s = S_(stream);
    dim3 grid(C / 32, count);
#define TFM(TA, NR_) hipLaunchKernelGGL((colbn_train_fwd_multi_kernel<TA, bf16, NR_>), grid, dim3(256), 0, s, m, momentum, eps, relu, \
                                        groups, (int)M, C)
    if (adtype == 0) { if (M <= 512) TFM(float, 8); else TFM(float, 16); }
    else             { if (M <= 512) TFM(bf16, 8); else TFM(bf16, 16); }
#undef TFM
    ASSL_LAUNCH_CHECK();
}

extern "C" int audiossl_colbn_bwd_multi(int count, int adtype, int gdtype, const void* const* a, const void* const* dh,
                                        const float* const* stats, int relu, int groups, long M, int C, void* const* da,
                                        float* const* dgamma, float* const* dbeta, void* stream) {
    ASSL_REQUIRE(count >= 1 && count <= MAXP && a && dh && stats && da && groups > 0 && M > 0 && M <= 1024 && C > 0 && (C % 32) == 0);
    ASSL_REQUIRE((adtype == 0 || adtype == 1) && (gdtype == 0 || gdtype == 1));
    BnBwdMulti m{};
    for (int p = 0; p < count; ++p) {
        ASSL_REQUIRE(a[p] && dh[p] && stats[p] && da[p]);
        m.a[p] = a[p]; m.dh[p] = dh[p]; m.st[p] = stats[p]; m.da[p] = da[p];
        m.dgamma[p] = dgamma ? dgamma[p] : nullptr; m.dbeta[p] = dbeta ? dbeta[p] : nullptr;
        ASSL_REQUIRE((m.dgamma[p] == nullptr) == (m.dbeta[p] == nullptr));
    }
// ... 367 lines not shown
```

audio-ssl_amd/src/engine.py:

```python
import os

import torch

from src import _native as N

import os as _os
_STEM_VALU = _os.environ.get("AUDIOSSL_STEM_VALU") == "1"
BN_MOMENTUM = 0.1
BN_EPS = 1e-5
_BN_FUSED = _os.environ.get("AUDIOSSL_BN_FUSED", "1") != "0"


ONE_STREAM = os.environ.get("AUDIOSSL_ONE_STREAM", "0") == "1"


_CAPTURE_ORIGIN = []


class capture_scope:

    def __enter__(self):
        _CAPTURE_ORIGIN.append(torch.cuda.current_stream())
        return self

# ... 90 lines not shown
def fast_copy(dst, src):
    n = src.numel()
    if src.dtype == torch.float32 and dst.dtype == torch.float32 and src.is_contiguous() and dst.is_contiguous() and n % 1024 == 0 \
            and n // 1024 < (1 << 31) and src.data_ptr() % 16 == 0 and dst.data_ptr() % 16 == 0:
        N.call("tile_rows", src, dst, n // 1024, n // 1024, 1, 1.0, 1024)
    else:
        dst.copy_(src)
    return dst


def _ksplit(M, Nn, K, target=512):
    tiles = ((M + 127) // 128) * ((Nn + 127) // 128)
    return int(max(1, min(target // max(tiles, 1), (K // 64) // 32)))


def gemm(dtype, ta, tb, M, Nn, K, A, lda, B, ldb, C, ldc, alpha=1.0, bias=None, relu=0, keep=None, ldk=0, keep_scale=1.0,
         gate=None, ldg=0, out_f32=0, atomic=0, ksplit=1, resid=None, ldr=0):
    N.call("gemm", dtype, ta, tb, M, Nn, K, float(alpha), A, lda, B, ldb, C, ldc, bias, relu, keep, ldk, float(keep_scale),
           gate, ldg, out_f32, atomic, ksplit, resid, ldr)


def linear_fwd(dtype, X, W, M, Nout, K, bias=None, relu=0, keep=None, keep_scale=1.0, out=None, out_f32=0):
    if out is None and dtype == N.BF16 and out_f32 and not relu and keep is None and M * Nout <= (1 << 16) and K >= 1024 and K % 512 == 0:
        out = ARENA.zeros((M, Nout), torch.float32, like=X)
        gemm(dtype, 0, 0, M, Nout, K, X, K, W, K, out, Nout, bias=bias, out_f32=1, atomic=1, ksplit=min(8, K // 256))
        return out
    if out is None:
        out = _empty((M, Nout), torch.float32 if (out_f32 or dtype == 0) else torch.bfloat16, like=X)
    gemm(dtype, 0, 0, M, Nout, K, X, K, W, K, out, Nout, bias=bias, relu=relu, keep=keep, ldk=Nout, keep_scale=keep_scale,
         out_f32=out_f32)
    return out


def linear_bwd_w(dtype, dY, X, dW, M, Nout, K, dw_zero=False):
    ks = _ksplit(Nout, K, M)
    atomic = 1 if (ks > 1 or dtype != N.BF16) else (0 if dw_zero else 2)
    gemm(dtype, 1, 1, Nout, K, M, dY, Nout, X, K, dW, K, out_f32=1, atomic=atomic, ksplit=ks)


def linear_bwd_x(dtype, dY, W, M, Nout, K, alpha=1.0, gate=None, out=None, out_f32=0):
    if out is None:
        out = _empty((M, K), torch.float32 if (out_f32 or dtype == N.F32) else torch.bfloat16, like=dY)
    gemm(dtype, 0, 1, M, K, Nout, dY, Nout, W, K, out, K, alpha=alpha, gate=gate, ldg=K, out_f32=out_f32)
    return out


GD = N.F32

HP = False


def set_high_precision(flag):
    global HP
    HP = bool(flag)


SYNC_BN = None


class SyncBN:
    def __init__(self, group=None):
        import torch.distributed as dist
        self.dist, self.group = dist, group
        self.world = dist.get_world_size(group)

    def all_reduce(self, t):
        self.dist.all_reduce(t, group=self.group)
        return t


def set_sync_bn(sync):
    global SYNC_BN
    SYNC_BN = sync if (sync is not None and sync.world > 1) else None


def _ad(dtype):
    return N.F32 if (HP or dtype == N.F32) else dtype


def pooled_dtype(dtype):
    return torch.float32


def center_cast(Y, groups, B):
    C = Y.shape[1]
    yc = _empty((groups * B, C), torch.bfloat16, like=Y)
    cmean = _empty((groups, C), torch.float32, like=Y)
    N.call("center_cast", Y, yc, cmean, groups, B, C)
    return yc, cmean


def colsum_add(dtype, X, M, C, dst, tmp=None):
    tmp = tmp if tmp is not None else ARENA.scratch((C,), torch.float64, X)
    N.call("colstats", dtype, X, 1, M, C, C, 0, tmp, None)
    N.call("add_d2f", tmp, dst, C)


def cast(dtype, src, n=None):
    if dtype == N.F32:
        return src
    out = torch.empty(src.shape, dtype=torch.bfloat16, device=src.device)
    N.call("cast", dtype, src, out, src.numel())
    return out


class EncoderCtx:
    pass


def _bn_train(dtype, Y, M, C, gamma, beta, rm, rv, update_running, groups=1):
    sq = ARENA.scratch((2, groups * C), torch.float64, Y)
    N.call("colstats", dtype, Y, groups, M, C, C, 1, sq[0], sq[1])
    if SYNC_BN is not None:
        SYNC_BN.all_reduce(sq)
        M = M * SYNC_BN.world
    st = _empty((4, groups * C), torch.float32, like=Y)
    N.call("bn_finalize", sq[0], sq[1], groups, float(M), C, gamma, beta, rm if update_running else None,
           rv if update_running else None, BN_MOMENTUM, BN_EPS, st[0], st[1], st[2], st[3])
    return st[0], st[1], st[2], st[3]


def bn_train_apply(dtype, ad, a, M, C, gamma, beta, rm, rv, update_running, groups, relu, out):
    if M <= 1024 and C % 32 == 0 and _BN_FUSED and SYNC_BN is None:
        st = _empty((4, groups * C), torch.float32, like=a)
        N.call("colbn_train_fwd", dtype, ad, a, gamma, beta, rm if update_running else None, rv if update_running else None,
               BN_MOMENTUM, BN_EPS, relu, groups, M, C, out, st[0], st[1], st[2], st[3])
        return st[0], st[1], st[2], st[3]
    st = _bn_train(ad, a, M, C, gamma, beta, rm, rv, update_running, groups)
    N.call("colbn_fwd", dtype, ad, a, st[0], st[1], relu, out, groups, M, C)
    return st


def _bn_eval(like, C, gamma, beta, rm, rv):
    scale, shift = _empty((C,), torch.float32, like=like), _empty((C,), torch.float32, like=like)
    N.call("bn_eval_affine", gamma, beta, rm, rv, BN_EPS, C, scale, shift)
    return scale, shift


_WGRAD_WS = {}


def _wgrad_workspace(device):
    key = device.index if device.index is not None else torch.cuda.current_device()
    ws = _WGRAD_WS.get(key)
    if ws is None:
        ws = _WGRAD_WS[key] = torch.empty(256 * 64 * 576, dtype=torch.float32, device=device)
    return ws


STAT_REPLICAS = 8
LOSS_REPLICAS = 32
_BN_STATS_P = os.environ.get("AUDIOSSL_BN_STATS_P", "1") != "0"
_DP1_BF16 = os.environ.get("AUDIOSSL_DP1_BF16", "1") != "0"


def _conv_block_fwd(dtype, Pin, Nimg, Ti, Fi, W, bias, bn, train, update_running, col, packed=None):
    td = N.torch_dtype(dtype)
    if packed is not None:
        Wf, Wd = packed
    else:
        Wf, Wd = _empty((64, 576), td, like=Pin), _empty((64, 576), td, like=Pin)
        N.call("pack_conv_w", dtype, W, Wf, Wd)
    M = Nimg * Ti * Fi
    ad = _ad(dtype)
    Y = _empty((M, 64), N.torch_dtype(ad), like=Pin)
    gamma, beta, rm, rv = bn
    fused = dtype == N.BF16 and Fi in (16, 32)
    rep = STAT_REPLICAS if (fused and train and SYNC_BN is None) else 1
    sq = ARENA.scratch((rep, 2, 64), torch.float64, Pin) if (fused and train) else None
    if fused:
        N.call("conv3x3_fwd", Pin, Wf, bias, Y, int(ad == N.F32), None if sq is None else sq[0, 0], None if sq is None else sq[0, 1],
               rep, Nimg, Ti, Fi)
    else:
        N.call("im2col3x3", dtype, Pin, col, Nimg, Ti, Fi)
        gemm(dtype, 0, 0, M, 64, 576, col, 576, Wf, 576, Y, 64, bias=bias, out_f32=int(ad == N.F32))
    Pout = _empty((Nimg, Ti // 2, Fi // 2, 64), td, like=Pin)
    if train and fused and SYNC_BN is None:
        st = _empty((4, 64), torch.float32, like=Pin)
        N.call("bn_relu_pool_train_fwd", dtype, ad, Y, sq[0, 0], sq[0, 1], rep, float(M), gamma, beta, rm if update_running else None,
               rv if update_running else None, BN_MOMENTUM, BN_EPS, Pout, st[0], st[1], st[2], st[3], Nimg, Ti, Fi)
        return Y, Pout, (st[0], st[1], st[2], st[3]), Wf, Wd
    if train and fused:
        st = _empty((4, 64), torch.float32, like=Pin)
        sq = sq[0]
        SYNC_BN.all_reduce(sq)
        N.call("bn_finalize", sq[0], sq[1], 1, float(M * SYNC_BN.world), 64, gamma, beta, rm if update_running else None,
               rv if update_running else None, BN_MOMENTUM, BN_EPS, st[0], st[1], st[2], st[3])
        scale, shift, mean, rstd = st[0], st[1], st[2], st[3]
    elif train:
        scale, shift, mean, rstd = _bn_train(ad, Y, M, 64, gamma, beta, rm, rv, update_running)
    else:
        scale, shift = _bn_eval(Y, 64, gamma, beta, rm, rv)
        mean = rstd = None
    N.call("bn_relu_pool_fwd", dtype, ad, Y, scale, shift, Pout, Nimg, Ti, Fi)
    return Y, Pout, (scale, shift, mean, rstd), Wf, Wd


def _col_buffer(dtype, Nimg, T1, F1, like):
    if dtype == N.BF16 and F1 in (16, 32):
        return None
    return _empty((Nimg * T1 * F1, 576), N.torch_dtype(dtype), like=like)


MOM_SLOT = 17 * 54


def stem_fused(dtype, train=True):
    return bool(train) and dtype == N.BF16 and not HP and not _STEM_VALU and SYNC_BN is None


def stem_moments_pair(xa, xb=None):
    Nimg, _, F, T = xa.shape
    assert xb is None or xb.shape == xa.shape
    mom = ARENA.scratch((1 if xb is None else 2, MOM_SLOT), torch.float64, xa)
    N.call("conv1_moments_pair", xa.reshape(Nimg, F, T).contiguous(), None if xb is None else xb.reshape(Nimg, F, T).contiguous(),
           Nimg, F, T, mom)
    return mom


def encoder_forward(P, x, dtype, keep=None, p_drop=0.3, train=True, update_running=True, want_layers=True, Wc=None,
                    layer_out=None, before_fc=None, stem_moments=None):
    Nimg, _, F, T = x.shape
    assert F == 64, "the HIP encoder is built for n_mels = 64 (the reference's only setting)"
    td = N.torch_dtype(dtype)
    c = EncoderCtx()
    c.P = P
    c.dtype, c.N, c.F, c.T, c.train, c.p_drop = dtype, Nimg, F, T, train, p_drop
    img = x.reshape(Nimg, F, T).contiguous()
    c.img = img
    w1 = P["features_1.0.weight"].reshape(64, 9)
    b1 = P["features_1.0.bias"]
    g1, be1 = P["features_1.1.weight"], P["features_1.1.bias"]
    c.stem_mfma = dtype == N.BF16 and not HP and not _STEM_VALU
    fused = stem_fused(dtype, train)
    assert stem_moments is None or fused, "precomputed stem moments are for the fused bf16 training stem only"
    rm1 = rv1 = None
    if train:
        c.sc1, c.sh1, c.mean1, c.rstd1 = (_empty((64,), torch.float32, like=x) for _ in range(4))
        rm1 = P["features_1.1.running_mean"] if update_running else None
        rv1 = P["features_1.1.running_var"] if update_running else None
    if fused:
        c.mom1 = stem_moments if stem_moments is not None else stem_moments_pair(x)[0]
    elif train:
        c.mom1 = ARENA.scratch((16 * 54,), torch.float64, x)
        if SYNC_BN is None:
            N.call("conv1_stats", img, Nimg, F, T, w1, b1, g1, be1, rm1, rv1, BN_MOMENTUM, BN_EPS, c.mom1, c.sc1, c.sh1, c.mean1, c.rstd1)
        else:
            N.call("conv1_moments", img, Nimg, F, T, c.mom1)
            mom_g = SYNC_BN.all_reduce(c.mom1[:54].clone())
            N.call("conv1_finalize", mom_g, w1, b1, g1, be1, rm1, rv1, BN_MOMENTUM, BN_EPS, float(Nimg * F * T * SYNC_BN.world),
                   c.sc1, c.sh1, c.mean1, c.rstd1)
    else:
        c.sc1, c.sh1 = _bn_eval(x, 64, g1, be1, P["features_1.1.running_mean"], P["features_1.1.running_var"])
    T1, F1 = T // 2, F // 2
    c.P1 = _empty((Nimg, T1, F1, 64), td, like=x)
    x1 = x2 = x3 = None
    if want_layers:
        x1, x2, x3 = layer_out if layer_out is not None else (_empty((Nimg, f * 64), td, like=x) for f in (F // 2, F // 4, F // 8))
    x1_fused = c.stem_mfma and x1 is not None and x1.dtype == torch.float32 and x1.is_contiguous()
    x1_parts = _empty((4, Nimg, (F // 2) * 64), torch.float32, like=x) if x1_fused else None
    if fused:
        N.call("conv1_fwd_train", img, Nimg, F, T, c.mom1, float(Nimg * F * T), w1, b1, g1, be1, rm1, rv1, BN_MOMENTUM, BN_EPS,
               c.sc1, c.sh1, c.mean1, c.rstd1, c.P1, x1_parts)
    else:
        N.call("conv1_fwd", dtype if (dtype == N.F32 or c.stem_mfma) else 2, img, Nimg, F, T, w1, b1, c.sc1, c.sh1, c.P1, x1_parts)
    col = _col_buffer(dtype, Nimg, T1, F1, x)
    bn2 = (P["features_2.1.weight"], P["features_2.1.bias"], P["features_2.1.running_mean"], P["features_2.1.running_var"])
    packs = [_empty((64, 576), td, like=x) for _ in range(4)]
    N.call("pack_conv_w2", dtype, P["features_2.0.weight"], packs[0], packs[1], P["features_3.0.weight"], packs[2], packs[3])
    c.Y2, c.P2, c.st2, c.W2f, c.W2d = _conv_block_fwd(dtype, c.P1, Nimg, T1, F1, P["features_2.0.weight"],
                                                       P["features_2.0.bias"], bn2, train, update_running, col, packed=packs[:2])
    T2, F2 = T1 // 2, F1 // 2
    bn3 = (P["features_3.1.weight"], P["features_3.1.bias"], P["features_3.1.running_mean"], P["features_3.1.running_var"])
    c.Y3, c.P3, c.st3, c.W3f, c.W3d = _conv_block_fwd(dtype, c.P2, Nimg, T2, F2, P["features_3.0.weight"],
                                                       P["features_3.0.bias"], bn3, train, update_running, col, packed=packs[2:])
    del col
    T3, F3 = T2 // 2, F2 // 2
    c.dims = (T1, F1, T2, F2, T3, F3)
    if want_layers:
        o32 = int(x1.dtype == torch.float32)
        N.call("tmean3_fwd", dtype, o32, None if x1_fused else c.P1, x1, x1_parts, T1, F1, c.P2, x2, T2, F2, c.P3, x3, T3, F3, Nimg)
    d = P["fc.0.weight"].shape[0]
    kin = F3 * 64
    M = Nimg * T3
    c.d, c.kin, c.M = d, kin, M
    if before_fc is not None:
        before_fc()
    if Wc is not None:
        c.fw1, c.fw2 = Wc["fc.0.weight"], Wc["fc.3.weight"]
    else:
        c.fw1, c.fw2 = cast(dtype, P["fc.0.weight"]), cast(dtype, P["fc.3.weight"])
    if keep is not None and not isinstance(keep, torch.Tensor) and (dtype != N.BF16 or not train):
        keep = keep.materialise()
    c.keep = keep if train else None
    scale = 1.0 / (1.0 - p_drop) if c.keep is not None else 1.0
    if c.keep is not None and not isinstance(c.keep, torch.Tensor):
        vk = c.keep
        c.H1 = torch.empty(M, d, dtype=torch.bfloat16, device=c.P3.device)
        N.call("gemm_dropout", 0, 0, M, d, kin, 1.0, c.P3, kin, c.fw1, kin, c.H1, d, P["fc.0.bias"], 1, vk.seed, float(vk.p), vk.counter,
               float(scale))
    else:
        c.H1 = linear_fwd(dtype, c.P3, c.fw1, M, d, kin, bias=P["fc.0.bias"], relu=1, keep=c.keep, keep_scale=scale)
    c.H2 = linear_fwd(dtype, c.H1, c.fw2, M, d, d, bias=P["fc.3.bias"], relu=1)
    return x1, x2, x3, c.H2.view(Nimg, T3, d), c


def _conv_block_bwd(dtype, Y, dP, dxl, st, Nimg, Ti, Fi, Pin, Wd, G_w, G_gamma, G_beta, need_dx, col, keep, dx_bf16=False, Pout=None):
    td = N.torch_dtype(dtype)
    scale, shift, mean, rstd = st
    M = Nimg * Ti * Fi
    dY = torch.empty((M, 64), dtype=td, device=Y.device)
    stat = ARENA.scratch((33 * 128,), torch.float32, Y)
    yd = N.F32 if Y.dtype == torch.float32 else dtype
    if SYNC_BN is None and Pout is not None and _BN_STATS_P and Pout.dtype == td:
        N.call("bn_relu_pool_bwd_p", dtype, yd, GD, Y, Pout, dP, dxl, scale, shift, mean, rstd, stat, dY, G_gamma, G_beta, Nimg, Ti, Fi)
    elif SYNC_BN is None:
        N.call("bn_relu_pool_bwd", dtype, yd, GD, Y, dP, dxl, scale, shift, mean, rstd, stat, dY, G_gamma, G_beta, Nimg, Ti, Fi)
    else:
        N.call("bn_relu_pool_bwd_stats", dtype, yd, GD, Y, dP, dxl, scale, shift, mean, rstd, stat, Nimg, Ti, Fi)
        gstat = SYNC_BN.all_reduce(stat[:128].clone())
        N.call("bn_relu_pool_bwd_apply", dtype, yd, GD, Y, dP, dxl, scale, shift, mean, rstd, stat, gstat, float(M * SYNC_BN.world), dY,
               G_gamma, G_beta, Nimg, Ti, Fi)
    fused = dtype == N.BF16 and Fi in (16, 32)
    if fused:
        def wg():
            dWp = ARENA.zeros((64, 576), torch.float32, device=Y.device)
            ws = _wgrad_workspace(Y.device)
            N.call("conv3x3_wgrad", dY, Pin, dWp, ws, ws.numel(), Nimg, Ti, Fi)
            N.call("unpack_conv_dw", dWp, G_w)
            return dWp
        keep.append((dY, WGRAD.run(Y.device, wg)))
    else:
        dWp = ARENA.zeros((64, 576), torch.float32, device=Y.device)
        N.call("im2col3x3", dtype, Pin, col, Nimg, Ti, Fi)
        gemm(dtype, 1, 1, 64, 576, M, dY, 64, col, 576, dWp, 576, out_f32=1, atomic=1, ksplit=_ksplit(64, 576, M, 1024))
        N.call("unpack_conv_dw", dWp, G_w)
    if not need_dx:
        return None
    dx_bf16 = dx_bf16 and fused
    dPin = _empty((Nimg, Ti, Fi, 64), torch.bfloat16 if dx_bf16 else torch.float32, like=Y)
    if fused:
        N.call("conv3x3_fwd", dY, Wd, None, dPin, 0 if dx_bf16 else 1, None, None, 1, Nimg, Ti, Fi)
    else:
        N.call("im2col3x3", dtype, dY, col, Nimg, Ti, Fi)
        gemm(dtype, 0, 0, M, 64, 576, col, 576, Wd, 576, dPin, 64)
    return dPin


def encoder_backward(c, G, dA2=None, dH2=None, dx1=None, dx2=None, dx3=None, dx_late=None, grads_zero=False):
    dtype, Nimg, M, d, kin = c.dtype, c.N, c.M, c.d, c.kin
    T1, F1, T2, F2, T3, F3 = c.dims
    td = N.torch_dtype(dtype)
    assert c.train, "backward needs a train-mode forward (batch statistics)"
    if dA2 is None:
        dA2 = _empty((M, d), td, like=c.H2)
        N.call("relu_bwd", dtype, dH2.contiguous(), c.H2, dA2, M * d)
    dev = c.H2.device
    def w2():
        linear_bwd_w(dtype, dA2, c.H1, G["fc.3.weight"], M, d, d, dw_zero=grads_zero)
        colsum_add(dtype, dA2, M, d, G["fc.3.bias"])
    WGRAD.run(dev, w2)
    scale = 1.0 / (1.0 - c.p_drop) if c.keep is not None else 1.0
    dA1 = linear_bwd_x(dtype, dA2, c.fw2, M, d, d, alpha=scale, gate=c.H1)
    def w1():
        linear_bwd_w(dtype, dA1, c.P3, G["fc.0.weight"], M, d, kin, dw_zero=grads_zero)
        colsum_add(dtype, dA1, M, d, G["fc.0.bias"])
    WGRAD.run(dev, w1)
    dP3 = linear_bwd_x(dtype, dA1, c.fw1, M, d, kin, out_f32=1)
    if dx_late is not None:
        dx1, dx2, dx3 = dx_late()
    col = _col_buffer(dtype, Nimg, T1, F1, c.H2)
    keep = []
    dP2 = _conv_block_bwd(dtype, c.Y3, dP3, dx3, c.st3, Nimg, T2, F2, c.P2, c.W3d, G["features_3.0.weight"],
                          G["features_3.1.weight"], G["features_3.1.bias"], True, col, keep, Pout=c.P3)
    dP1 = _conv_block_bwd(dtype, c.Y2, dP2, dx2, c.st2, Nimg, T1, F1, c.P1, c.W2d, G["features_2.0.weight"],
                          G["features_2.1.weight"], G["features_2.1.bias"], True, col, keep, dx_bf16=bool(c.stem_mfma) and _DP1_BF16,
                          Pout=c.P2)
    gd1 = N.BF16 if dP1.dtype == torch.bfloat16 else GD
    acc = ARENA.scratch((32 * 64 * 11,), torch.float32, c.H2)
    P = c.P
    w1, b1, g1 = P["features_1.0.weight"].reshape(64, 9), P["features_1.0.bias"], P["features_1.1.weight"]
    gw, gb = G["features_1.0.weight"].view(64, 9), G["features_1.0.bias"]
    if SYNC_BN is None:
        N.call("conv1_bwd", gd1, int(c.stem_mfma), c.img, Nimg, c.F, c.T, w1, b1, g1, c.sc1, c.sh1, c.mean1, c.rstd1, c.mom1, dP1, dx1,
               acc, gw, gb, G["features_1.1.weight"], G["features_1.1.bias"])
    else:
        lstat = _empty((128,), torch.float32, like=c.H2)
        N.call("conv1_bwd_sums", gd1, int(c.stem_mfma), c.img, Nimg, c.F, c.T, w1, b1, g1, c.sc1, c.sh1, c.mean1, c.rstd1, c.mom1, dP1,
               dx1, acc, lstat)
        gstat = SYNC_BN.all_reduce(lstat.clone())
        N.call("conv1_bwd_finalize", acc, c.mom1, w1, b1, g1, c.mean1, c.rstd1, float(Nimg * c.F * c.T * SYNC_BN.world), gstat, gw, gb,
               G["features_1.1.weight"], G["features_1.1.bias"])
    WGRAD.join(dev)


def maxmean_forward(dtype, H2, out=None):
    Nimg, T3, d = H2.shape
    y = out if out is not None else _empty((Nimg, d), N.torch_dtype(dtype), like=H2)
    arg = _empty((Nimg, d), torch.uint8, like=H2)
    N.call("maxmean_fwd", dtype, int(y.dtype == torch.float32), H2, y, arg, Nimg, T3, d)
    return y, arg


def maxmean_backward(dtype, dy, arg, H2):
    Nimg, T3, d = H2.shape
    dA2 = _empty((Nimg * T3, d), N.torch_dtype(dtype), like=H2)
    N.call("maxmean_bwd", dtype, GD, dy, arg, H2, dA2, Nimg, T3, d)
    return dA2


class ProjCtx:
    pass


def projector_forward(PP, Y, dtype, groups, B, update_running=True, Wc=None):
    kin = Y.shape[1]
    c = ProjCtx()
    c.dtype, c.B, c.groups, c.kin, c.y = dtype, B, groups, kin, Y
    W = Wc if Wc is not None else tuple(cast(dtype, PP[f"projector.{i}.weight"]) for i in (0, 3, 6))
    c.W = W
    D = W[0].shape[0]
    c.D = D
    M = groups * B

    def bn(a, prefix, affine, relu, out, adt=None):
        g = PP[prefix + ".weight"] if affine else None
        b = PP[prefix + ".bias"] if affine else None
        return bn_train_apply(dtype, ad if adt is None else adt, a, B, D, g, b, PP[prefix + ".running_mean"], PP[prefix + ".running_var"],
                              update_running, groups, relu, out)
    td = N.torch_dtype(dtype)
    ad = _ad(dtype)
    c.ad = ad
    o32 = int(ad == N.F32)
    c.cmean = None
    if dtype == N.BF16 and Y.dtype == torch.float32 and not HP and B <= 1024 and kin % 32 == 0 and SYNC_BN is None:
        c.y_hi, c.cmean = center_cast(Y, groups, B)
        c.y_lo = None
        c.a1 = linear_fwd(dtype, c.y_hi, W[0], M, D, kin, out_f32=o32)
    elif dtype == N.BF16 and Y.dtype == torch.float32:
        c.y_hi, c.y_lo = _empty((M, kin), td, like=Y), _empty((M, kin), td, like=Y)
        N.call("split_bf16", Y, c.y_hi, c.y_lo, M * kin)
        c.a1 = torch.zeros(M, D, dtype=torch.float32, device=Y.device)
        gemm(dtype, 0, 0, M, D, kin, c.y_hi, kin, W[0], kin, c.a1, D, out_f32=1, atomic=1)
        gemm(dtype, 0, 0, M, D, kin, c.y_lo, kin, W[0], kin, c.a1, D, out_f32=1, atomic=1)
    else:
        c.y_hi, c.y_lo = Y, None
        c.a1 = linear_fwd(dtype, Y, W[0], M, D, kin, out_f32=o32)
    c.ad1 = N.F32 if c.a1.dtype == torch.float32 else ad
    c.h1 = _empty((M, D), td, like=Y)
    c.st1 = bn(c.a1, "projector.1", True, 1, c.h1, adt=c.ad1)
    if c.cmean is not None and update_running:
        N.call("shift_running_mean", W[0], c.cmean, PP["projector.1.running_mean"], D, kin, groups, BN_MOMENTUM)
    c.a2 = linear_fwd(dtype, c.h1, W[1], M, D, D, out_f32=o32)
    c.h2 = _empty((M, D), td, like=Y)
    c.st2 = bn(c.a2, "projector.4", True, 1, c.h2)
    c.z = linear_fwd(dtype, c.h2, W[2], M, D, D, out_f32=o32)
    c.zn = _empty((M, D), td, like=Y)
    c.st0 = bn(c.z, "bn", False, 0, c.zn)
    return c.zn, c


def projector_backward(c, PP, G, dzn, dy_rows=None):
    dtype, B, D, kin, groups = c.dtype, c.B, c.D, c.kin, c.groups
    M = groups * B
    td = N.torch_dtype(dtype)

    def bn_bwd(a, dh, st, relu, da, g_gamma, g_beta, adt=None):
        adt = c.ad if adt is None else adt
        """BatchNorm1d(train) backward per group (view).  SyncBatchNorm (`extras/delores-s/main.py:79` converts every BatchNorm of
        the model, the projector's included): the two means of the backward are over the GLOBAL batch of the view - this rank's
        sums are all-reduced between the statistics pass and the apply pass; the parameter gradients stay this rank's own sums
        (the data-parallel gradient all-reduce adds the ranks up afterwards)."""
        t = ARENA.scratch((2 * groups * D,), torch.float64, dzn)
        if SYNC_BN is None:
            N.call("colbn_bwd", dtype, adt, GD, a, dh, *st, relu, groups, B, D, t, da, g_gamma, g_beta)
            return
        N.call("colbn_bwd_stats", dtype, adt, GD, a, dh, *st, relu, groups, B, D, t)
        tg = SYNC_BN.all_reduce(t.clone())
        N.call("colbn_bwd_apply", dtype, adt, GD, a, dh, *st, relu, groups, B, D, tg, float(B * SYNC_BN.world), da)
        if g_gamma is not None:
            for g in range(groups):
                N.call("add_d2f", t[g * D:(g + 1) * D], g_beta, D)
                N.call("add_d2f", t[(groups + g) * D:(groups + g + 1) * D], g_gamma, D)
    dz = _empty((M, D), td, like=c.zn)
    bn_bwd(c.z, dzn, c.st0, 0, dz, None, None)
    linear_bwd_w(dtype, dz, c.h2, G["projector.6.weight"], M, D, D)
    dh2 = linear_bwd_x(dtype, dz, c.W[2], M, D, D, out_f32=1)
    da2 = _empty((M, D), td, like=c.zn)
    bn_bwd(c.a2, dh2, c.st2, 1, da2, G["projector.4.weight"], G["projector.4.bias"])
    linear_bwd_w(dtype, da2, c.h1, G["projector.3.weight"], M, D, D)
    dh1 = linear_bwd_x(dtype, da2, c.W[1], M, D, D, out_f32=1)
    da1 = _empty((M, D), td, like=c.zn)
    bn_bwd(c.a1, dh1, c.st1, 1, da1, G["projector.1.weight"], G["projector.1.bias"], adt=c.ad1)
    linear_bwd_w(dtype, da1, c.y_hi, G["projector.0.weight"], M, D, kin)
    if c.y_lo is not None:
        linear_bwd_w(dtype, da1, c.y_lo, G["projector.0.weight"], M, D, kin)
    rows = M if dy_rows is None else dy_rows
    if rows == 0:
        return None
    return linear_bwd_x(dtype, da1, c.W[0], rows, D, kin, out_f32=1)


def barlow_forward_backward(PP, G, Y, dtype, lambd, scale_loss, loss_out, need_dy1=True, need_dy2=True,
                            update_running=True, all_reduce=None, global_batch=None, backward=True, Wc=None):
    B = Y.shape[0] // 2
    zn, c = projector_forward(PP, Y, dtype, 2, B, update_running, Wc)
    D = c.D
    zn1, zn2 = zn[:B], zn[B:]
    denom = float(global_batch if global_batch else B)
    cmat = _empty((D, D), torch.float32, like=Y)
    gemm(dtype, 1, 1, D, D, B, zn1, D, zn2, D, cmat, D, alpha=1.0 / denom, out_f32=1)
    if all_reduce is not None:
        all_reduce(cmat)
    coef = (lambd if lambd else 1.0) * scale_loss
    dc = _empty((D, D), N.torch_dtype(dtype), like=Y)
    N.call("barlow_loss", dtype, cmat, D, coef, 2.0 * coef / denom, dc, loss_out)
    if not backward:
        return None
    dzn = _empty((2 * B, D), torch.float32, like=Y)
    gemm(dtype, 0, 0, B, D, D, zn2, D, dc, D, dzn[:B], D, out_f32=1)
    gemm(dtype, 0, 1, B, D, D, zn1, D, dc, D, dzn[B:], D, out_f32=1)
    rows = 2 * B if need_dy2 else (B if need_dy1 else 0)
    return projector_backward(c, PP, G, dzn, rows)


def _harr(ctype, xs):
    import ctypes
    vals = [x.data_ptr() if isinstance(x, torch.Tensor) else x for x in xs]
    return (ctype * len(vals))(*vals)


def _multi_check(*lists):
    for ts in lists:
        for t in ts:
            if t is not None and (not t.is_cuda or not t.is_contiguous()):
                raise RuntimeError("multi-problem launches need contiguous device tensors")


def gemm_multi(ta, tb, M, Nn, Ks, As, ldas, Bs, ldbs, Cs, ldc, alpha=1.0, out_f32=0, atomic=0, ksplit=1):
    import ctypes
    n = len(As)
    _multi_check(As, Bs, Cs)
    Ns = [Nn] * n if isinstance(Nn, int) else list(Nn)
    ldcs = [ldc] * n if isinstance(ldc, int) else list(ldc)
    adr = ctypes.addressof
    arrs = (_harr(ctypes.c_int, Ns), _harr(ctypes.c_int, Ks), _harr(ctypes.c_void_p, As), _harr(ctypes.c_long, ldas),
            _harr(ctypes.c_void_p, Bs), _harr(ctypes.c_long, ldbs), _harr(ctypes.c_void_p, Cs), _harr(ctypes.c_long, ldcs))
    N_, K_, A_, la_, B_, lb_, C_, lc_ = arrs
    if N.PROFILE is not None:
        N.PROFILE_NOTE = float(sum(2.0 * M * nn * kk for nn, kk in zip(Ns, Ks)))
    N.call("gemm_multi", n, ta, tb, M, adr(N_), adr(K_), float(alpha), adr(A_), adr(la_), adr(B_), adr(lb_), adr(C_), adr(lc_),
           out_f32, atomic, ksplit)


def gemm_multi_sgd(ta, tb, M, Nn, Ks, As, ldas, Bs, ldbs, Ps, Moms, Shadows, ldp, hyper, alpha=1.0):
    import ctypes
    n = len(As)
    _multi_check(As, Bs, Ps, Moms, [] if Shadows is None else Shadows)
    Ns = [Nn] * n if isinstance(Nn, int) else list(Nn)
# ... 177 lines not shown
```

audio-ssl_amd/src/upstream/delores_m/upstream_expert.py:

```python
import os

import torch
import torch.nn as nn

from src import _native as N
from src import engine as E
from src.encoder.audiontt import default_precision
from src.flat import FlatGroup
from src.module_base import UpstreamModule
from src.upstream.common import EAGER, FusedExpertMixin, FusedStepFn, MocoQueueMixin, Projection, strip
from src.upstream.delores_m.upstream_encoder import DELORES_M as DELORES_M_ENCODER
from src.utils import concat_all_gather


_PREP_ASIDE = os.environ.get("AUDIOSSL_PREP_ASIDE", "1") != "0"
_HEADS_ASIDE = os.environ.get("AUDIOSSL_HEADS_ASIDE", "1") != "0"
_FUSED_SGD = os.environ.get("AUDIOSSL_FUSED_SGD", "1") != "0"
_SKIP_ZERO = os.environ.get("AUDIOSSL_SKIP_ZERO", "1") != "0"
_GRADS_ZERO = os.environ.get("AUDIOSSL_GRADS_ZERO", "1") != "0"
_DY_EVENT = os.environ.get("AUDIOSSL_DY_EVENT", "1") != "0"
_LATE_JOIN = os.environ.get("AUDIOSSL_LATE_JOIN", "1") != "0"
_SGD_ASIDE = os.environ.get("AUDIOSSL_SGD_ASIDE", "1") != "0"
_STEM_PAIR = os.environ.get("AUDIOSSL_STEM_PAIR", "0") == "1"

# ... 19 lines not shown
        self.datamodule = datamodule
        self.encoder_q, self.encoder_k = self.init_encoders(self.base_encoder)
        for param_q, param_k in zip(self.encoder_q.parameters(), self.encoder_k.parameters()):
            param_k.data.copy_(param_q.data)
            param_k.requires_grad = False
        self.register_buffer("queue", nn.functional.normalize(torch.randn(emb_dim, num_negatives), dim=0))
        self.register_buffer("queue_ptr", torch.zeros(1, dtype=torch.long))
        lam, scale = self.config["pretrain"]["lambda_barlow"], self.config["pretrain"]["loss_scale"]
        self.p1 = Projection(2048, lam[0], scale)
        self.p2 = Projection(1024, lam[1], scale)
        self.p3 = Projection(512, lam[2], scale)
        prec = config.get("run", {}).get("precision")
        self.precision = {"fp32": N.F32, "bf16": N.BF16, "bf16_hp": N.BF16}.get(prec, default_precision())
        self.high_precision = prec == "bf16_hp"
        self.grouped_heads = bool(config.get("run", {}).get("grouped_heads", os.environ.get("AUDIOSSL_GROUPED_HEADS", "1") != "0"))
        self.encoder_q.encoder.precision = self.encoder_k.encoder.precision = self.precision
        self.flat_k = None
        self._key_stream = E.SideStream()
        self._prep_stream = E.SideStream()

    def init_encoders(self, base_encoder):
        return DELORES_M_ENCODER(self.config, base_encoder), DELORES_M_ENCODER(self.config, base_encoder)

    def trainable_named(self):
        named = [(n, p) for n, p in self.named_parameters() if n.startswith("encoder_q.")]
        named += [(n, p) for n, p in self.named_parameters() if n.startswith(("p1.", "p2.", "p3."))]
        return named

    def fused_loss(self, img_q, img_k, need_grad=True, parts=None, runner=None, optimizer=None):
        with E.ARENA.step(img_q.device):
            return self._fused_loss(img_q, img_k, need_grad, parts, runner, optimizer)

    def _fused_loss(self, img_q, img_k, need_grad, parts, runner, optimizer):
        R = runner or EAGER
        dt = self.precision
        E.set_high_precision(self.high_precision)
        flat = self.ensure_flat()
        dev = img_q.device
        B = img_q.shape[0]
        eq, ek = self.encoder_q, self.encoder_k
        ddp = _world() > 1
        img_k = img_k.float().contiguous()
        img_q = img_q.float().contiguous()
        pending_k = self._shuffle_begin(img_k) if ddp else None
        main = torch.cuda.current_stream()
        G = flat.grad_dict
        Ys = R.alloc("Ys", lambda: [torch.empty(2 * B, f, dtype=E.pooled_dtype(dt), device=dev) for f in (2048, 1024, 512)])

        moms = None
        if _STEM_PAIR and not ddp and E.stem_fused(dt, self.training):
            moms = R.phase("stem_moments", lambda: E.stem_moments_pair(img_q, img_k))
            if not E.ONE_STREAM:
                moms.record_stream(self._key_stream.stream(dev))

        def key_phase(x):
            self._momentum_update_key_encoder(shadow_dtype=dt)
            self.flat_k.refresh_shadow(dt)
            Wk = self.flat_k.shadow_dict()
            keepk = ek.encoder.next_keep_mask(B, x.shape[-1])
            _, _, _, Hk, _ = E.encoder_forward(ek.encoder.param_dict(), x, dt, keep=keepk, p_drop=0.3, train=self.training,
                                               Wc=strip(Wk, "encoder."), layer_out=tuple(y[B:] for y in Ys),
                                               stem_moments=None if moms is None else moms[1])
            yk, _ = E.maxmean_forward(dt, Hk)
            wk = Wk["fc.weight"]
            return E.linear_fwd(dt, yk, wk, B, wk.shape[0], wk.shape[1], bias=ek.fc.bias.data, out_f32=1)

        def key_branch():
            x, idx_unshuffle = img_k, None
            if ddp:
                x, idx_unshuffle = self._shuffle_end(pending_k, B)
                x = R.static("key_in", x)
            kk = R.phase("key", lambda: key_phase(x))
            if ddp:
                kk = R.static("key_out", self._batch_unshuffle_ddp(kk, idx_unshuffle))
            return kk
        k = self._key_stream.run(dev, key_branch)

        heads = (self.p1, self.p2, self.p3)
        grouped = not (self.high_precision or dt == N.F32 or not self.grouped_heads or E.SYNC_BN is not None)
        D_ = self.p1.param_dict()["projector.3.weight"].shape[0]
        kins_ = [p.param_dict()["projector.0.weight"].shape[1] for p in heads]
        stored_grads = tuple(f"p{i + 1}.projector.{j}.weight" for i in range(3) for j in (0, 3, 6)) \
            if (need_grad and grouped and _GRADS_ZERO and _SKIP_ZERO and E.heads_wgrads_store(D_, kins_, 2 * B)) else ()

        sgd_ctx = None
        if stored_grads and _FUSED_SGD and optimizer is not None and not ddp and hasattr(optimizer, "fused_wgrad"):
            sgd_ctx = optimizer.fused_wgrad(flat, [f"p{i + 1}." for i in range(3)])

        def query_phase():
            def prep():
                if need_grad:
                    flat.zero_grad(stores_ok=bool(stored_grads))
                flat.refresh_shadow(dt)
            busy = (need_grad and not (flat._fresh_grad is True or (flat._fresh_grad == "partial" and stored_grads))) or \
                   not (flat._fresh_shadow or dt == N.F32)
            if _PREP_ASIDE and busy:
                self._prep_stream.run(dev, prep)
            else:
                prep()
            Wq = flat.shadow_dict("encoder_q.")
            wq = Wq["fc.weight"]
            fold = not (self.high_precision or dt == N.F32 or not self.grouped_heads)
            loss = torch.zeros(4 + (3 * E.LOSS_REPLICAS if fold else 0), dtype=torch.float32, device=dev)
            keep = eq.encoder.next_keep_mask(B, img_q.shape[-1])
            _, _, _, Hq, cq = E.encoder_forward(eq.encoder.param_dict(), img_q, dt, keep=keep, p_drop=0.3, train=self.training,
                                                Wc=strip(Wq, "encoder."), layer_out=tuple(y[:B] for y in Ys),
                                                before_fc=(lambda: self._prep_stream.join(dev)) if (_PREP_ASIDE and busy) else None,
                                                stem_moments=None if moms is None else moms[0])
            yq, argq = E.maxmean_forward(dt, Hq)
            q = E.linear_fwd(dt, yq, wq, B, wq.shape[0], wq.shape[1], bias=eq.fc.bias.data, out_f32=1)
            return loss, wq, Hq, cq, yq, argq, q
        loss, wq, Hq, cq, yq, argq, q = R.phase("query", query_phase)
        self._key_stream.join(dev)
        k.record_stream(main)

        streams = self._streams(dev)
        dys = [None, None, None]
        dy_event = None

        def head_phase(i, p):
            Wp = flat.shadow_dict(f"p{i + 1}.")
            return E.barlow_forward_backward(p.param_dict(), G(f"p{i + 1}."), Ys[i], dt, p.lambd, p.scale_loss,
                                             loss[i + 1:i + 2], need_dy1=True, need_dy2=False,
                                             update_running=self.training, backward=need_grad,
                                             Wc=tuple(Wp[f"projector.{j}.weight"] for j in (0, 3, 6)))
        if not grouped:
            for i, p in enumerate(heads):
                if not E.ONE_STREAM:
                    E.fork(streams[i], main)
                with torch.cuda.stream(streams[i]):
                    dys[i] = R.phase(f"head{i + 1}", lambda i=i, p=p: head_phase(i, p))
        else:
            def heads_phase():
                Wps = [flat.shadow_dict(f"p{i + 1}.") for i in range(3)]
                return E.barlow_heads_forward_backward(
                    [p.param_dict() for p in heads], [G(f"p{i + 1}.") for i in range(3)], Ys, dt, [p.lambd for p in heads],
                    [p.scale_loss for p in heads],
                    [loss[4 + i * E.LOSS_REPLICAS:4 + (i + 1) * E.LOSS_REPLICAS] for i in range(3)], update_running=self.training,
                    backward=need_grad, Wcs=[tuple(Wp[f"projector.{j}.weight"] for j in (0, 3, 6)) for Wp in Wps],
                    grads_zero=need_grad and _GRADS_ZERO,
                    dy_ready=(lambda: dy_event.record()) if dy_event is not None else None, sgd=sgd_ctx)
            hs = streams[0] if _HEADS_ASIDE else main
            if not E.ONE_STREAM and _HEADS_ASIDE:
                E.fork(streams[0], main)
            if need_grad and not ddp and not E.ONE_STREAM and _HEADS_ASIDE and _SGD_ASIDE and _DY_EVENT:
                dy_event = torch.cuda.Event()
            with torch.cuda.stream(hs):
                dys = list(R.phase("heads", heads_phase))

        def moco_phase():
            shadow = self.queue_shadow(dt)
            dq, kn32 = E.moco_forward_backward(dt, q, k, self.queue, shadow, float(self.hparams.softmax_temperature),
                                               loss[0:1], backward=need_grad)
            dA2 = None
            if need_grad:
                Gq = G("encoder_q.")
                E.linear_bwd_w(dt, dq, yq, Gq["fc.weight"], B, wq.shape[0], wq.shape[1])
                E.colsum_add(dt, dq, B, wq.shape[0], Gq["fc.bias"])
                dyq = E.linear_bwd_x(dt, dq, wq, B, wq.shape[0], wq.shape[1], out_f32=1)
                dA2 = E.maxmean_backward(dt, dyq, argq, Hq)
            return kn32, dA2
        kn32, dA2 = R.phase("moco", moco_phase)
        self._dequeue_and_enqueue(kn32, self.queue_shadow(dt) if dt != N.F32 else None)
        early_box = [None]

        def join_heads():
            for i, st in enumerate(streams):
                if E.ONE_STREAM:
                    continue
                if i == 0 and dy_event is not None:
                    main.wait_event(dy_event)
                else:
                    main.wait_stream(st)
            for d in dys:
                if d is not None:
                    d.record_stream(main)
            if not need_grad:
                return dys
            self.reduce_begin("heads")
            if optimizer is not None and not ddp and hasattr(optimizer, "step_tail"):
                early = streams[0] if _SGD_ASIDE else main
                if not E.ONE_STREAM and _SGD_ASIDE and dy_event is None:
                    E.fork(early, main)
                with torch.cuda.stream(early):
                    if R.phase("sgd_heads", lambda: optimizer.step_tail(flat, self.head_offset(), stored=stored_grads,
                                                                        stepped=sgd_ctx is not None)):
                        optimizer.mark_early(flat, self.head_offset())
                        early_box[0] = early
                    elif sgd_ctx is not None:
                        raise RuntimeError("the projector weights were stepped by their weight-gradient GEMMs but the head-segment "
                                           "SGD pass declined: the optimiser's step() would step them again")
            return dys

        late = need_grad and not ddp and _LATE_JOIN
        if not late:
            join_heads()
        if need_grad:
            def backward_phase():
                if late:
                    box = [None]

                    def join_and_sum():
                        d = join_heads()
                        box[0] = loss.sum()
                        return d
                    E.encoder_backward(cq, G("encoder_q.encoder."), dA2=dA2, dx_late=join_and_sum, grads_zero=_GRADS_ZERO)
                    return box[0]
                E.encoder_backward(cq, G("encoder_q.encoder."), dA2=dA2, dx1=dys[0], dx2=dys[1], dx3=dys[2],
                                   grads_zero=_GRADS_ZERO)
                return loss.sum()
            total = R.phase("encoder_bwd", backward_phase)
            if early_box[0] is not None and not E.ONE_STREAM and _SGD_ASIDE:
                main.wait_stream(early_box[0])
            elif dy_event is not None:
                main.wait_stream(streams[0])
            self.reduce_begin("enc")
        else:
            total = loss.sum()
        if parts is not None:
            parts["losses"] = loss if loss.numel() == 4 else torch.cat([loss[:1], loss[4:].view(3, E.LOSS_REPLICAS).sum(1)])
        return total

    def _streams(self, dev):
        if E.ONE_STREAM:
            return [torch.cuda.current_stream(dev)] * 3
        if getattr(self, "_side_streams", None) is None or self._side_streams[0].device != dev:
            self._side_streams = [torch.cuda.Stream(device=dev) for _ in range(3)]
        return self._side_streams

    def forward(self, img_q=None, img_k=None):
        raise NotImplementedError("the HIP expert fuses forward and loss; call training_step((img_1, img_2), i)")

    def training_step(self, batch, batch_idx):
        img_1, img_2 = batch
        params = self.ensure_flat().params
        loss = FusedStepFn.apply(self, torch.is_grad_enabled(), img_1, img_2, *params)
        self.log_dict({'train_loss': loss})
        return loss
```

include/audiossl_hip.h:

```cpp
#ifndef AUDIOSSL_HIP_H
#define AUDIOSSL_HIP_H

#include <stdint.h>

#ifdef __cplusplus
extern "C" {
#endif

#define AUDIOSSL_OK 0
#define AUDIOSSL_EINVAL (-1)
#define AUDIOSSL_ELAUNCH (-2)
#define AUDIOSSL_EALIGN (-3)

int audiossl_logmel_fwd(const float* wave, float* out, int B, int L, int T, int n_fft, int hop, int n_mels, int taps,
                        const float* win, const float* tw, const float* melw, const int* mel_start, float eps_pow,
                        float eps_log, int apply_log, void* stream);

int audiossl_fbank_fwd(const float* wave, const int* lens, const int* partner, const float* lam, float* clip_mean,
                       const int* bands, const int* bands_host, float* out, int B, int Lmax, int win_len, int shift, int n_fft, int n_mels,
                       int taps, int T_target, const float* win, const float* tw, const float* melw, const int* mel_start,
                       float preemph, float eps_log, float mean, float std, int skip_norm, int time_major, void* stream);

int audiossl_clip_moments(const float* x, double* mom, int B, int n, void* stream);
int audiossl_runnorm_scan(const double* mom, int B, int n_elem, long long* state_i, float* state_f, float* mu_out,
                          float* sd_out, void* stream);
int audiossl_aug_normalize(const float* x, const float* mu, const float* sd, float* bank, long slot0, int R, int B, int n,
                           void* stream);
int audiossl_aug_views(const float* bank, int R, const int* ip, const float* fp, float* out1, float* out2, int B, int F,
                       int T, int canvas_h, int canvas_w, int log_mix, void* stream);
int audiossl_aug_plan_host(uint32_t* np_key, int* np_pos, uint32_t* py_key, int* py_pos, int B, int F, int T,
                           long long clips_seen, long long* n_entries, int R, int n_memory, int use_mix, double ratio,
                           int use_rrc, double fs_lo, double fs_hi, double ts_lo, double ts_hi, int canvas_h,
                           int canvas_w, int use_spec, int spec_F, int spec_T, int spec_nf, int spec_nt, const int* lens,
                           int unit, int* starts, int* ip, float* fp, int* masks);

int audiossl_resample_sinc(const float* x, float* y, int clips, int n_orig, int n_out, const int* n, const int* off_l,
                           const int* off_r, const double* eta_l, const double* eta_r, const double* win, const double* delta,
                           int nwin, int index_step, void* stream);

int audiossl_pcm_window(const void* pcm, long pcm_bytes, const long long* tab, const long long* tab_host, float* out, int B,
                        int unit, int align, void* stream);

int audiossl_kmix_cluster(const float* views, const float* centroids, int n_views, int F, int T, int K, int* cluster,
                          void* stream);
int audiossl_kmix_apply(const float* views, const float* ring, const int* slot, const float* coef, int n_views, int n,
                        int log_mix, float* out, void* stream);
int audiossl_mask_fill(float* x, const int* tab, int n_img, int max_masks, int F, int T, int zero_fill, void* stream);

int audiossl_conv1_stats(const float* img, int N, int F, int T, const float* w, const float* bias, const float* gamma,
                         const float* beta, float* running_mean, float* running_var, float momentum, float eps,
                         double* mom, float* scale, float* shift, float* save_mean, float* save_rstd, void* stream);
#define AUDIOSSL_CONV1_XL_PARTS 4
int audiossl_conv1_fwd(int dtype, const float* img, int N, int F, int T, const float* w, const float* bias,
                       const float* scale, const float* shift, void* out, float* xl, void* stream);
#define AUDIOSSL_CONV1_MOM_SLOT (17 * 54)
int audiossl_conv1_moments_pair(const float* img_a, const float* img_b, int N, int F, int T, double* mom, void* stream);
int audiossl_conv1_fwd_train(const float* img, int N, int F, int T, double* mom, double count, const float* w, const float* bias,
                             const float* gamma, const float* beta, float* running_mean, float* running_var, float momentum,
                             float eps, float* scale, float* shift, float* save_mean, float* save_rstd, void* out, float* xl,
                             void* stream);
int audiossl_conv1_bwd(int dtype, int conv_dtype, const float* img, int N, int F, int T, const float* w, const float* bias,
                       const float* gamma, const float* scale, const float* shift, const float* mean, const float* rstd,
                       const double* mom, const void* dP, const void* dxl, float* acc, float* dW, float* dbias,
                       float* dgamma, float* dbeta, void* stream);

int audiossl_colstats(int dtype, const void* x, int groups, long M, int C, long ld, int want_sq, double* sum,
                      double* sumsq, void* stream);
int audiossl_bn_finalize(const double* sum, const double* sumsq, int groups, double count, int C, const float* gamma,
                         const float* beta, float* running_mean, float* running_var, float momentum, float eps,
                         float* scale, float* shift, float* save_mean, float* save_rstd, void* stream);
int audiossl_bn_relu_pool_fwd(int dtype, int ydtype, const void* Y, const float* scale, const float* shift, void* P, int N,
                              int Ti, int Fi, void* stream);
int audiossl_bn_relu_pool_train_fwd(int dtype, int ydtype, const void* Y, const double* sum, const double* sumsq, int stat_replicas,
                                    double count, const float* gamma, const float* beta, float* running_mean, float* running_var,
                                    float momentum, float eps, void* P, float* scale, float* shift, float* save_mean, float* save_rstd,
                                    int N, int Ti, int Fi, void* stream);
int audiossl_tmean_fwd(int dtype, int out_f32, const void* P, void* xl, int N, int To, int Fo, void* stream);
int audiossl_tmean3_fwd(int dtype, int out_f32, const void* P1, void* x1, const float* x1_parts, int To1, int Fo1, const void* P2,
                        void* x2, int To2, int Fo2, const void* P3, void* x3, int To3, int Fo3, int N, void* stream);
int audiossl_bn_relu_pool_bwd(int dtype, int ydtype, int gdtype, const void* Y, const void* dP, const void* dxl, const float* scale,
                              const float* shift, const float* mean, const float* rstd, float* stat, void* dY,
                              float* dgamma, float* dbeta, int N, int Ti, int Fi, void* stream);
int audiossl_bn_relu_pool_bwd_p(int dtype, int ydtype, int gdtype, const void* Y, const void* P, const void* dP, const void* dxl,
                                const float* scale, const float* shift, const float* mean, const float* rstd, float* stat, void* dY,
                                float* dgamma, float* dbeta, int N, int Ti, int Fi, void* stream);
int audiossl_conv1_moments(const float* img, int N, int F, int T, double* mom, void* stream);
int audiossl_conv1_finalize(double* mom_totals, const float* w, const float* bias, const float* gamma, const float* beta,
                            float* running_mean, float* running_var, float momentum, float eps, double count, float* scale,
                            float* shift, float* save_mean, float* save_rstd, void* stream);
int audiossl_conv1_bwd_sums(int dtype, int conv_dtype, const float* img, int N, int F, int T, const float* w, const float* bias,
                            const float* gamma, const float* scale, const float* shift, const float* mean, const float* rstd,
                            const double* mom, const void* dP, const void* dxl, float* acc, float* lstat, void* stream);
int audiossl_conv1_bwd_finalize(const float* acc, const double* mom, const float* w, const float* bias, const float* gamma,
                                const float* mean, const float* rstd, double count_global, const float* gstat, float* dW,
                                float* dbias, float* dgamma, float* dbeta, void* stream);
int audiossl_bn_relu_pool_bwd_stats(int dtype, int ydtype, int gdtype, const void* Y, const void* dP, const void* dxl,
                                    const float* scale, const float* shift, const float* mean, const float* rstd, float* stat,
                                    int N, int Ti, int Fi, void* stream);
int audiossl_bn_relu_pool_bwd_apply(int dtype, int ydtype, int gdtype, const void* Y, const void* dP, const void* dxl,
                                    const float* scale, const float* shift, const float* mean, const float* rstd, float* stat,
                                    const float* gstat, double count_global, void* dY, float* dgamma, float* dbeta, int N, int Ti,
                                    int Fi, void* stream);
int audiossl_colbn_bwd_stats(int dtype, int adtype, int gdtype, const void* a, const void* dh, const float* scale,
                             const float* shift, const float* mean, const float* rstd, int relu, int groups, long M, int C,
                             double* tmp, void* stream);
int audiossl_colbn_bwd_apply(int dtype, int adtype, int gdtype, const void* a, const void* dh, const float* scale,
                             const float* shift, const float* mean, const float* rstd, int relu, int groups, long M, int C,
                             const double* sums, double count, void* da, void* stream);
int audiossl_im2col3x3(int dtype, const void* X, void* col, int N, int Ti, int Fi, void* stream);
int audiossl_pack_conv_w(int dtype, const float* W, void* Wf, void* Wd, void* stream);
int audiossl_pack_conv_w2(int dtype, const float* Wa, void* Wfa, void* Wda, const float* Wb, void* Wfb, void* Wdb, void* stream);
int audiossl_unpack_conv_dw(const float* dWp, float* dW, void* stream);

int audiossl_conv3x3_fwd(const void* X, const void* W, const float* bias, void* Y, int out_f32, double* sum,
                         double* sumsq, int stat_replicas, int N, int Ti, int Fi, void* stream);
int audiossl_conv3x3_wgrad(const void* dY, const void* X, float* dWp, float* workspace, long workspace_floats, int N, int Ti,
                           int Fi, void* stream);

int audiossl_gemm(int dtype, int trans_a, int trans_b, int M, int N, int K, float alpha, const void* A, long lda,
                  const void* B, long ldb, void* C, long ldc, const float* bias, int relu, const uint8_t* keep, long ldk,
                  float keep_scale, const void* gate, long ldg, int out_f32, int atomic, int ksplit, const float* resid,
                  long ldr, void* stream);

int audiossl_gemm_dropout(int trans_a, int trans_b, int M, int N, int K, float alpha, const void* A, long lda, const void* B,
                          long ldb, void* C, long ldc, const float* bias, int relu, unsigned long long seed, float p,
                          const long long* counter, float keep_scale, void* stream);

int audiossl_gemm_multi(int count, int trans_a, int trans_b, int M, const int* N, const int* K, float alpha,
                        const void* const* A, const long* lda, const void* const* B, const long* ldb, void* const* C,
                        const long* ldc, int out_f32, int atomic, int ksplit, void* stream);
int audiossl_gemm_multi_sgd(int count, int trans_a, int trans_b, int M, const int* Nv, const int* K, float alpha,
                            const void* const* A, const long* lda, const void* const* B, const long* ldb, float* const* P,
                            float* const* Mom, void* const* Shadow, const long* ldp, float lr, float momentum, float weight_decay,
                            float grad_scale, const float* grad_scale_dev, void* stream);
int audiossl_gemm_multi_barlow(int count, int D, const int* K, float alpha, const void* const* A, const long* lda,
                               const void* const* B, const long* ldb, void* const* dc, const float* coef, const float* dscale,
                               float* const* loss_rep, void* stream);

int audiossl_maxmean_fwd(int dtype, int out_f32, const void* H, void* y, uint8_t* arg, int N, int Tt, int D, void* stream);
int audiossl_maxmean_bwd(int dtype, int gdtype, const void* dy, const uint8_t* arg, const void* H, void* dA, int N, int Tt,
                         int D, void* stream);

int audiossl_colbn_fwd(int dtype, int adtype, const void* a, const float* scale, const float* shift, int relu, void* h,
                       int groups, long M, int C, void* stream);
int audiossl_colbn_train_fwd(int dtype, int adtype, const void* a, const float* gamma, const float* beta,
                             float* running_mean, float* running_var, float momentum, float eps, int relu, int groups,
                             long M, int C, void* h, float* scale, float* shift, float* save_mean, float* save_rstd,
                             void* stream);
int audiossl_colbn_bwd(int dtype, int adtype, int gdtype, const void* a, const void* dh, const float* scale, const float* shift, const float* mean,
                       const float* rstd, int relu, int groups, long M, int C, double* tmp, void* da, float* dgamma,
                       float* dbeta, void* stream);
int audiossl_colbn_train_fwd_multi(int count, int adtype, const void* const* a, const float* const* gamma,
                                   const float* const* beta, float* const* running_mean, float* const* running_var,
                                   float momentum, float eps, int relu, int groups, long M, int C, void* const* h,
                                   float* const* stats, void* stream);
int audiossl_colbn_bwd_multi(int count, int adtype, int gdtype, const void* const* a, const void* const* dh,
                             const float* const* stats, int relu, int groups, long M, int C, void* const* da,
                             float* const* dgamma, float* const* dbeta, void* stream);
int audiossl_barlow_loss_multi(int count, const float* const* c, int D, const float* coef, const float* dscale,
                               void* const* dc, float* const* loss_out, void* stream);
int audiossl_add_d2f(const double* src, float* dst, int n, void* stream);
int audiossl_barlow_loss(int dtype, const float* c, int D, float coef, float dscale, void* dc, float* loss_out,
                         void* stream);

int audiossl_l2norm_fwd(int dtype, const float* q, int B, int D, void* qn, float* qn32, float* inv_norm, void* stream);
int audiossl_moco_prep(int dtype, const float* q, const float* k, int B, int D, float scale, void* qn, float* qn32, float* qinv,
                       void* kn, float* kn32, float* kinv, float* lpos, void* stream);
int audiossl_rowdot(const float* a, const float* b, int B, int D, float scale, float* out, void* stream);
int audiossl_moco_ce_fwd(const float* lpos, const float* lneg, int B, int K, float* lse, float* loss_out, void* stream);
int audiossl_moco_ce_bwd(int dtype, const float* lpos, const float* lneg, const float* lse, int B, int K, float gscale,
                         void* P, float* dlpos, void* stream);
int audiossl_moco_logits(int mode, const void* qn, const void* queue, int B, int K, int dim, float inv_t, float* part,
                         const float* lse, float gscale, void* P, void* stream);
int audiossl_moco_lse_merge(const float* lpos, const float* part, int B, int nslot, float gscale, float* lse,
                            float* loss_out, float* dlpos, void* stream);
int audiossl_l2norm_bwd(int dtype, const float* dqn, const float* dlpos, const float* kn32, const float* qn32,
                        const float* inv_norm, int B, int D, void* dq, void* stream);
int audiossl_enqueue(int dtype, const float* keys, int B, int D, int K, int ptr, long long* ptr_dev, float* queue, void* shadow,
                     void* stream);
int audiossl_ema_update(float* pk, const float* pq, long n, float m, void* shadow, void* stream);

int audiossl_set_prezeroed(int on);
int audiossl_last_kernel(char* name, int capacity);

int audiossl_sgd_momentum(float* p, float* g, float* buf, long n, float lr, float momentum, float weight_decay,
                          int first, float grad_scale, const float* grad_scale_dev, void* shadow_bf16, int zero_grad,
                          void* stream);
int audiossl_sgd_momentum_segments(float* p, float* g, float* buf, const long* segs, int nseg, long max_n, float lr, float momentum,
                                   float weight_decay, int first, float grad_scale, const float* grad_scale_dev, void* shadow_bf16,
                                   int zero_grad, void* stream);
int audiossl_zero_segments(float* g, const long* segs, int nseg, long max_n, void* stream);
int audiossl_cast(int dtype, const float* src, void* dst, long n, void* stream);
int audiossl_cast_back(int dtype, const void* src, float* dst, long n, void* stream);
int audiossl_dropout_mask(uint8_t* keep, long n, unsigned long long seed, float p, const long long* counter, void* stream);
int audiossl_relu_bwd(int dtype, const void* g, const void* h, void* out, long n, void* stream);
int audiossl_bn_eval_affine(const float* gamma, const float* beta, const float* running_mean, const float* running_var,
                            float eps, int C, float* scale, float* shift, void* stream);
int audiossl_axpy(float* y, const float* x, float a, long n, void* stream);
int audiossl_split_bf16(const float* x, void* hi, void* lo, long n, void* stream);
int audiossl_center_cast(const float* y, void* yc, float* cmean, int groups, long M, int C, void* stream);
int audiossl_shift_running_mean(const void* W, const float* cmean, float* running_mean, int D, int K, int groups,
                                float momentum, void* stream);
int audiossl_center_cast_multi(int count, const float* const* y, void* const* yc, float* const* cmean, const int* C, int groups,
                               long M, void* stream);
int audiossl_shift_running_mean_multi(int count, const void* const* W, const float* const* cmean, float* const* running_mean,
                                      int D, const int* K, int groups, float momentum, void* stream);

int audiossl_ntxent_fwd(const float* sim, int N, int B, float* lse, float* loss_out, void* stream);
int audiossl_ntxent_bwd(int dtype, const float* sim, const float* lse, int N, int B, float gscale, void* dsim, void* stream);

int audiossl_row_argmax(const float* dot, long N, int K, long long* assign, void* stream);
int audiossl_kmeans_accumulate(const float* x, const long long* assign, long N, int K, int D, float* sums, int* counts,
                               void* stream);
int audiossl_kmeans_update(const float* sums, const int* counts, int K, int D, float* centroids, void* stream);
int audiossl_kmeans_update_mean(const float* sums, const int* counts, int K, int D, float* centroids, void* stream);
int audiossl_row_sqnorm(const float* x, int rows, int D, float scale, float* out, void* stream);
int audiossl_ce_rows(int dtype, const float* logits, const long long* target, int B, int K, int ignore_index, int* cnt,
                     float* loss_out, void* dlogits, void* stream);

int audiossl_softmax_rows_fwd(const float* x, float* y, int M, int C, void* stream);
int audiossl_softmax_rows_bwd(const float* y, const float* gy, float* gx, int M, int C, void* stream);

int audiossl_attn_fwd(const void* qkv, void* out, float* lse, int B, int S, int H, float scale, void* stream);
int audiossl_attn_bwd(const void* qkv, const void* out, const void* dout, const float* lse, void* dqkv, int B, int S, int H,
                      float scale, void* stream);
int audiossl_layernorm_fwd(const float* x, const float* gamma, const float* beta, void* y, float* y32, float* mean, float* rstd,
                           int M, int C, float eps, void* stream);
int audiossl_layernorm_bwd(const float* dy, const float* x, const float* mean, const float* rstd, const float* gamma,
                           float* dres, float* dgamma, float* dbeta, int M, int C, void* stream);
int audiossl_gelu_fwd(const void* a, void* h, long n, void* stream);
int audiossl_gelu_bwd(const void* a, const void* dh, void* da, long n, void* stream);
int audiossl_patch_unfold(const float* x, void* out, int B, int F, int T, int fstride, int tstride, void* stream);
int audiossl_tile_rows(const float* src, float* out, long rows, int period, int group, float scale, int C, void* stream);
int audiossl_adamw(float* p, const float* g, float* m, float* v, long n, float lr, float beta1, float beta2, float eps,
                   float weight_decay, float grad_scale, const long long* step, void* stream);

int audiossl_mvit_pool_fwd(const void* qkv, int ldq, int col0, const float* w, const float* gamma, const float* beta, float* out,
                           float* z, float* mean, float* rstd, int B, int heads, int d, int H, int W, int Ho, int Wo, int sh, int sw,
                           float eps, void* stream);
int audiossl_mvit_pool_bwd(const void* qkv, int ldq, int col0, const float* w, const float* gamma, const float* dout, const float* z,
                           const float* mean, const float* rstd, float* dz, float* dw, float* dgamma, float* dbeta, void* dqkv, int B,
                           int heads, int d, int H, int W, int Ho, int Wo, int sh, int sw, void* stream);
int audiossl_mvit_attn_fwd(const float* q, const float* k, const float* v, const float* rh, const float* rw, const int* ih,
                           const int* iw, void* out, float* lse, int B, int heads, int d, int qh, int qw, int kh, int kw, int nrh,
                           int nrw, int residual, float scale, void* stream);
int audiossl_mvit_attn_bwd(const float* q, const float* k, const float* v, const float* rh, const float* rw, const int* ih,
                           const int* iw, const void* dout, const float* lse, float* dq, float* dk, float* dv, float* drh, float* drw,
                           int B, int heads, int d, int qh, int qw, int kh, int kw, int nrh, int nrw, int residual, float scale,
                           void* stream);
int audiossl_tokpool_max_fwd(const float* x, float* y, void* arg, int B, int H, int W, int C, int kh, int kw, int sh, int sw,
                             void* stream);
int audiossl_tokpool_max_bwd(const float* dy, const void* arg, float* dx, int B, int H, int W, int C, int kh, int kw, int sh, int sw,
                             void* stream);

int audiossl_lars_step(float* p, const float* g, float* mu, const void* seg, int n_seg, const float* lr, float weight_decay,
                       float momentum, float eta, float grad_scale, double* norms, void* stream);
int audiossl_larc_step(float* p, const float* g, float* mu, const void* seg, int n_seg, float lr, float weight_decay,
                       float momentum, float trust_coefficient, float eps, int clip, float grad_scale, double* norms,
                       void* stream);

#ifdef __cplusplus
}
#endif
#endif
```

Measured before the change: 275,100 clips/s.

## Fuse BN-backward reductions into conv dgrad and maxmean backward epilogues

Adds a conv3x3 dgrad kernel variant for the 16-wide layer. While it produces the fp32 data gradient, it also accumulates the batch-norm backward sums (sum of dA and sum of dA times x-hat) for the next block down, so the separate stats pass over that activation can be skipped via a new apply-only phase. Separately, the maxmean backward kernel now produces the fc.3 bias column sums in the same pass, replacing a separate colsum kernel over dA2. Both cut extra full reads of large activations. The cost is more register and LDS pressure in the conv epilogue, extra loads of P and dxl there, and atomics.

New measurement: 277,100 clips/s, median of 6. No clear change (+0.7%).

```diff
diff --git a/audio-ssl_amd/csrc/bnpool.hip b/audio-ssl_amd/csrc/bnpool.hip
--- a/audio-ssl_amd/csrc/bnpool.hip
+++ b/audio-ssl_amd/csrc/bnpool.hip
@@ -545,19 +545,19 @@
     ASSL_REQUIRE(ydtype == 0 || ydtype == dtype);
     ASSL_REQUIRE(phase == 1 || (dY && dgamma && dbeta));
     hipStream_t s = static_cast<hipStream_t>(stream);
-    if (phase != 2) ASSL_ZERO(stat, sizeof(float) * 128 * 33, s);
+    if (phase < 2) ASSL_ZERO(stat, sizeof(float) * 128 * 33, s);
     const long total = (long)N * ((Ti + 1) / 2) * (Fi / 2) * 8;
     const int grid = ceil_div(total, 256);
     const float inv_To = 1.f / (float)(Ti / 2);
     const float inv_count = (float)(1.0 / (phase == 2 ? count : (double)N * Ti * Fi));
     float* apply_stat = phase == 2 ? const_cast<float*>(gstat) : stat;
-    const int fold = phase == 0;
+    const int fold = phase == 0 || phase == 3;
 #define BW(TY, AP, TG, TO, ST) hipLaunchKernelGGL((bn_relu_pool_bwd_kernel<TY, AP, TG, TO>), dim3(grid), dim3(256), 0, s,              \
         static_cast<const TY*>(Y), static_cast<const TG*>(dP), static_cast<const TG*>(dxl), inv_To, scale, shift, mean, rstd, ST, \
         inv_count, static_cast<TO*>(dY), N, Ti, Fi, (AP) ? fold : 0, dgamma, dbeta)
 #define BWP(TG, TO) hipLaunchKernelGGL((bn_pool_bwd_stats_p_kernel<TO, TG>), dim3(pgrid), dim3(256), 0, s, static_cast<const TO*>(P),          \
         static_cast<const TG*>(dP), static_cast<const TG*>(dxl), inv_To, scale, shift, mean, rstd, stat, N, Ti / 2, Fi / 2)
-#define BW2(TY, TG, TO) do { if (phase != 2) { if (P) BWP(TG, TO); else BW(TY, false, TG, TO, stat);                                       \
+#define BW2(TY, TG, TO) do { if (phase < 2) { if (P) BWP(TG, TO); else BW(TY, false, TG, TO, stat);                                       \
                                                if (!fold) hipLaunchKernelGGL(stat_reduce_kernel, dim3(1), dim3(128), 0, s, stat); }          \
                              if (phase != 1) BW(TY, true, TG, TO, apply_stat); } while (0)
     const long ptotal = (long)N * (Ti / 2) * (Fi / 2) * 8;
@@ -587,6 +587,13 @@
     return bn_relu_pool_bwd_run(0, dtype, ydtype, gdtype, Y, P, dP, dxl, scale, shift, mean, rstd, stat, nullptr, 0.0, dY, dgamma, dbeta, N,
                                 Ti, Fi, stream);
 }
+extern "C" int audiossl_bn_relu_pool_bwd_apply_sums(int dtype, int ydtype, int gdtype, const void* Y, const void* dP, const void* dxl,
+                                                    const float* scale, const float* shift, const float* mean, const float* rstd,
+                                                    float* stat, void* dY, float* dgamma, float* dbeta, int N, int Ti, int Fi,
+                                                    void* stream) {
+    return bn_relu_pool_bwd_run(3, dtype, ydtype, gdtype, Y, nullptr, dP, dxl, scale, shift, mean, rstd, stat, nullptr, 0.0, dY, dgamma, dbeta, N,
+                                Ti, Fi, stream);
+}
 extern "C" int audiossl_bn_relu_pool_bwd_stats(int dtype, int ydtype, int gdtype, const void* Y, const void* dP, const void* dxl,
                                                const float* scale, const float* shift, const float* mean, const float* rstd,
                                                float* stat, int N, int Ti, int Fi, void* stream) {
diff --git a/audio-ssl_amd/csrc/conv.hip b/audio-ssl_amd/csrc/conv.hip
--- a/audio-ssl_amd/csrc/conv.hip
+++ b/audio-ssl_amd/csrc/conv.hip
@@ -187,8 +187,15 @@
     static constexpr int BYTES = ROWS * COLS * 128;
 };
 
-template <int FI, bool STATS, bool F32OUT, int PF = 2>
-__global__ __launch_bounds__(256, 1) void conv3x3_ws_kernel(ConvArgs a) {
+struct BnSumArgs {
+    const bf16* P; const float* dxl; const float* scale; const float* shift; const float* mean; const float* rstd;
+    float* stat; float inv_T; int nimg;
+};
+constexpr int BNS_LDS_BYTES = 2 * 16 * 64 * 4 + 2 * 64 * 4;
+
+template <int FI, bool STATS, bool F32OUT, int PF, bool BNSUMS>
+__device__ __forceinline__ void conv3x3_ws_body(const ConvArgs& a, const BnSumArgs& b) {
+    static_assert(!BNSUMS || (F32OUT && !STATS && FI == 16), "BN-backward sums: fp32 data gradient of the 16-wide layer");
     using G = WsGeom<FI>;
     constexpr int TT = G::TT, COLS = G::COLS;
     typedef __attribute__((address_space(3))) void* lptr_t;
@@ -199,6 +206,8 @@
     char* const stg = reinterpret_cast<char*>(red + 4 * 64 * 2) + (threadIdx.x >> 6) * 64 * OPIX;
     char* const zblk = reinterpret_cast<char*>(red + 4 * 64 * 2) + 4 * 64 * OPIX;
     if (threadIdx.x < 32) *reinterpret_cast<f32x4*>(zblk + threadIdx.x * 16) = f32x4{0.f, 0.f, 0.f, 0.f};
+    char* const dxl_l = zblk + 512;
+    float* const bnk = reinterpret_cast<float*>(dxl_l + 2 * FI * 256);
 
     const int lane = threadIdx.x & 63, wave = __builtin_amdgcn_readfirstlane(threadIdx.x >> 6);
     const int m = lane & 31, h = lane >> 5;
@@ -276,6 +285,22 @@
         for (int e = 0; e < NS; ++e) { ssum[e] = 0.f; ssq[e] = 0.f; }
     }
 
+    const int c4 = lane & 15;
+    float bsum[4], bsx[4];
+    bf16x4 pv[2][8];
+    __amdgpu_buffer_rsrc_t rsrcx;
+    if constexpr (BNSUMS) {
+        if (threadIdx.x < 64) {
+            const int c = threadIdx.x;
+            const float sc = b.scale[c], inv = sc != 0.f ? 1.f / sc : 0.f;
+            bnk[c] = inv * b.rstd[c];
+            bnk[64 + c] = sc != 0.f ? -(b.shift[c] * inv + b.mean[c]) * b.rstd[c] : 0.f;
+        }
+#pragma unroll
+        for (int e = 0; e < 4; ++e) { bsum[e] = 0.f; bsx[e] = 0.f; }
+        rsrcx = __builtin_amdgcn_make_buffer_rsrc(const_cast<float*>(b.dxl), 0, b.dxl ? (unsigned)((long)b.nimg * FI * 256) : 0u, 0x00020000);
+    }
+
     int tile = blockIdx.x, cur = 0;
     if (tile < a.tiles) dma_tile(tile * TT, smem);
     asm volatile("s_waitcnt vmcnt(0) lgkmcnt(0)" ::: "memory");
@@ -290,6 +315,28 @@
         const int next = tile + gridDim.x;
         if (next < a.tiles && !(a.dbg & 2)) dma_tile(next * TT, smem + (cur ^ 1) * G::BYTES);
         const char* const hl = smem + cur * G::BYTES;
+        int n0 = 0;
+        if constexpr (BNSUMS) {
+            n0 = g0 / a.Ti;
+            if (b.dxl) {
+#pragma unroll
+                for (int k = 0; k < 2; ++k) {
+                    const int img = n0 + k < b.nimg ? n0 + k : b.nimg - 1;
+                    __builtin_amdgcn_raw_ptr_buffer_load_lds(rsrcx, (lptr_t)(dxl_l + k * (FI * 256) + wave * 1024), 16, lane * 16,
+                                                             img * (FI * 256) + wave * 1024, 0, 0);
+                }
+            }
+#pragma unroll
+            for (int i = 0; i < 2; ++i)
+#pragma unroll
+                for (int it = 0; it < 8; ++it) {
+                    const int p = it * 4 + (lane >> 4);
+                    const int row = g0 + (2 * wave + i) * (32 / FI) + (p / FI);
+                    const bf16 z = (bf16)0.f;
+                    pv[i][it] = row < a.rows_total ? *reinterpret_cast<const bf16x4*>(b.P + ((long)row * FI + (p % FI)) * CH + c4 * 4)
+                                                   : bf16x4{z, z, z, z};
+                }
+        }
 
         int bdt[2][3];
 #pragma unroll
@@ -339,8 +386,11 @@
         }
         if (ts) ts[tsi++] = __builtin_amdgcn_s_memtime();
         asm volatile("s_waitcnt vmcnt(0)" ::: "memory");
+        if constexpr (BNSUMS) { if (b.dxl) __builtin_amdgcn_s_barrier(); }
         if (ts) ts[tsi++] = __builtin_amdgcn_s_memtime();
         if (!(a.dbg & 1)) {
+            f32x4 bk1, bk0;
+            if constexpr (BNSUMS) { bk1 = *reinterpret_cast<const f32x4*>(bnk + c4 * 4); bk0 = *reinterpret_cast<const f32x4*>(bnk + 64 + c4 * 4); }
 #pragma unroll
             for (int i = 0; i < 2; ++i) {
                 char* const st = stg + i * 32 * OPIX;
@@ -372,6 +422,24 @@
                             if (STATS) {
 #pragma unroll
                                 for (int e = 0; e < 4; ++e) { ssum[e] += v[e]; ssq[e] += v[e] * v[e]; }
+                            }
+                            if constexpr (BNSUMS) {
+                                f32x4 g = v;
+                                if (b.dxl) {
+                                    const int n = (grow + p / FI) / a.Ti;
+                                    const f32x4 gx = n - n0 < 2
+                                        ? *reinterpret_cast<const f32x4*>(dxl_l + (n - n0) * (FI * 256) + (p % FI) * 256 + c4 * 16)
+                                        : *reinterpret_cast<const f32x4*>(b.dxl + (long)n * (FI * 64) + (p % FI) * 64 + c4 * 4);
+#pragma unroll
+                                    for (int e = 0; e < 4; ++e) g[e] += gx[e] * b.inv_T;
+                                }
+#pragma unroll
+                                for (int e = 0; e < 4; ++e) {
+                                    const float av = (float)pv[i][it][e];
+                                    const float da = av > 0.f ? g[e] : 0.f;
+                                    bsum[e] += da;
+                                    bsx[e] += da * (av * bk1[e] + bk0[e]);
+                                }
                             }
                         }
                     }
@@ -422,6 +490,36 @@
             atomicAdd(k == 0 ? &a.sum[rep + c] : &a.sumsq[rep + c], t);
         }
     }
+    if constexpr (BNSUMS) {
+#pragma unroll
+        for (int e = 0; e < 4; ++e) {
+            float s = bsum[e], q = bsx[e];
+#pragma unroll
+            for (int o = 16; o < 64; o <<= 1) { s += __shfl_xor(s, o, 64); q += __shfl_xor(q, o, 64); }
+            if (lane < 16) {
+                const int co = lane * 4 + e;
+                red[(wave * 64 + co) * 2] = s; red[(wave * 64 + co) * 2 + 1] = q;
+            }
+        }
+        __syncthreads();
+        if (threadIdx.x < 128) {
+            const int kind = threadIdx.x >> 6, c = threadIdx.x & 63;
+            float t = 0.f;
+#pragma unroll
+            for (int w = 0; w < 4; ++w) t += red[(w * 64 + c) * 2 + kind];
+            atomicAdd(&b.stat[128 + (blockIdx.x & 31) * 128 + kind * 64 + c], t);
+        }
+    }
+}
+
+template <int FI, bool STATS, bool F32OUT, int PF = 2>
+__global__ __launch_bounds__(256, 1) void conv3x3_ws_kernel(ConvArgs a) {
+    conv3x3_ws_body<FI, STATS, F32OUT, PF, false>(a, BnSumArgs{});
+}
+
+template <int FI>
+__global__ __launch_bounds__(256, 1) void conv3x3_dgrad_bnsums_kernel(ConvArgs a, BnSumArgs b) {
+    conv3x3_ws_body<FI, false, true, 2, true>(a, b);
 }
 
 __host__ __device__ __forceinline__ int wg_cot(int w, int n) { return n < 8 ? (n & 1) : (w & 1); }
@@ -639,6 +737,24 @@
     if (Fi == 32) { if (nw == 8) CONV_LAUNCH(32, 8, 0); else CONV_LAUNCH(32, 4, 1); }
     else          { if (nw == 8) CONV_LAUNCH(16, 8, 2); else CONV_LAUNCH(16, 4, 3); }
 #undef CONV_LAUNCH
+    ASSL_LAUNCH_CHECK();
+}
+
+extern "C" int audiossl_conv3x3_dgrad_bnsums(const void* dY, const void* W, void* dP, const void* P, const float* dxl,
+                                             const float* scale, const float* shift, const float* mean, const float* rstd,
+                                             float* stat, int N, int Ti, int Fi, void* stream) {
+    ASSL_REQUIRE(dY && W && dP && P && scale && shift && mean && rstd && stat && N > 0 && Ti > 0 && Fi == 16);
+    if (!ASSL_ALIGNED16(dY) || !ASSL_ALIGNED16(W) || !ASSL_ALIGNED16(dP) || !ASSL_ALIGNED16(P) || !ASSL_ALIGNED16(dxl)) return ASSL_EALIGN;
+    const int rows = N * Ti, TT = 256 / Fi, tiles = (rows + TT - 1) / TT;
+    ASSL_REQUIRE((long)rows * Fi * 128 < 0x7FFFFF00L);
+    hipStream_t s = static_cast<hipStream_t>(stream);
+    ASSL_ZERO(stat, sizeof(float) * 128 * 33, s);
+    ConvArgs a{static_cast<const bf16*>(dY), static_cast<const bf16*>(W), nullptr, static_cast<bf16*>(dP), nullptr, nullptr, Ti, rows, tiles, 1, 0, 1};
+    BnSumArgs b{static_cast<const bf16*>(P), dxl, scale, shift, mean, rstd, stat, 1.f / (float)Ti, N};
+    const size_t lds = 2 * WsGeom<16>::BYTES + sizeof(float) * (64 + 4 * 64 * 2) + 4 * 64 * 256 + 512 + BNS_LDS_BYTES;
+    static bool attr = false;
+    if (!attr) { if (set_lds(conv3x3_dgrad_bnsums_kernel<16>, lds)) return ASSL_ELAUNCH; attr = true; }
+    hipLaunchKernelGGL((conv3x3_dgrad_bnsums_kernel<16>), dim3(tiles < 256 ? tiles : 256), dim3(256), lds, s, a, b);
     ASSL_LAUNCH_CHECK();
 }
 
diff --git a/audio-ssl_amd/csrc/heads.hip b/audio-ssl_amd/csrc/heads.hip
--- a/audio-ssl_amd/csrc/heads.hip
+++ b/audio-ssl_amd/csrc/heads.hip
@@ -49,6 +49,51 @@
         o.set(i, h.get(i) > 0.f ? v : 0.f);
     }
     o.store(dA + idx * 8);
+}
+
+template <typename T_, typename TG>
+__global__ __launch_bounds__(1024) void maxmean_bwd_sums_kernel(const TG* __restrict__ dy, const uint8_t* __restrict__ arg,
+                                                                const T_* __restrict__ H, T_* __restrict__ dA,
+                                                                double* __restrict__ colsum, int N, int Tt, int D) {
+    __shared__ float red[16][512];
+    const int tx = threadIdx.x & 63, ty = threadIdx.x >> 6;
+    const int D8 = D / 8, d8 = blockIdx.x * 64 + tx;
+    const long M = (long)N * Tt, row0 = (long)blockIdx.y * 64;
+    const float inv = 1.f / (float)Tt;
+    float s[8];
+#pragma unroll
+    for (int i = 0; i < 8; ++i) s[i] = 0.f;
+#pragma unroll
+    for (int k = 0; k < 4; ++k) {
+        const long r = row0 + ty + 16 * k;
+        if (d8 < D8 && r < M) {
+            const int t = (int)(r % Tt);
+            const long n = r / Tt;
+            const Vec8<TG> g = Vec8<TG>::load(dy + n * D + d8 * 8);
+            const Vec8<T_> h = Vec8<T_>::load(H + (r * D8 + d8) * 8);
+            Vec8<T_> o;
+#pragma unroll
+            for (int i = 0; i < 8; ++i) {
+                const float gi = g.get(i);
+                const float v = gi * inv + (arg[n * D + d8 * 8 + i] == t ? gi : 0.f);
+                o.set(i, h.get(i) > 0.f ? v : 0.f);
+                s[i] += o.get(i);
+            }
+            o.store(dA + (r * D8 + d8) * 8);
+        }
+    }
+#pragma unroll
+    for (int i = 0; i < 8; ++i) red[ty][tx * 8 + i] = s[i];
+    __syncthreads();
+    if (threadIdx.x < 512) {
+        const int c = blockIdx.x * 512 + threadIdx.x;
+        if (c < D) {
+            double t = 0.0;
+#pragma unroll
+            for (int w = 0; w < 16; ++w) t += (double)red[w][threadIdx.x];
+            atomicAdd(&colsum[c], t);
+        }
+    }
 }
 
 template <typename TA, typename T_>
@@ -728,6 +773,20 @@
     if (dtype == 0) hipLaunchKernelGGL((maxmean_bwd_kernel<float, float>), GRID1(total), dim3(256), 0, S_(stream), (const float*)dy, arg, (const float*)H, (float*)dA, N, Tt, D);
     else if (gdtype == 0) hipLaunchKernelGGL((maxmean_bwd_kernel<bf16, float>), GRID1(total), dim3(256), 0, S_(stream), (const float*)dy, arg, (const bf16*)H, (bf16*)dA, N, Tt, D);
     else            hipLaunchKernelGGL((maxmean_bwd_kernel<bf16, bf16>), GRID1(total), dim3(256), 0, S_(stream), (const bf16*)dy, arg, (const bf16*)H, (bf16*)dA, N, Tt, D);
+    ASSL_LAUNCH_CHECK();
+}
+
+extern "C" int audiossl_maxmean_bwd_sums(int dtype, int gdtype, const void* dy, const uint8_t* arg, const void* H, void* dA,
+                                         double* colsum, int N, int Tt, int D, void* stream) {
+    ASSL_REQUIRE(dy && arg && H && dA && colsum && N > 0 && Tt > 0 && D > 0 && (D % 8) == 0 && (dtype == 0 || dtype == 1));
+    ASSL_REQUIRE(gdtype == 0 || gdtype == dtype);
+    const long M = (long)N * Tt;
+    ASSL_REQUIRE((M + 63) / 64 <= 65535);
+    ASSL_ZERO(colsum, sizeof(double) * D, S_(stream));
+    const dim3 grid(ceil_div(D, 512), ceil_div(M, 64));
+    if (dtype == 0) hipLaunchKernelGGL((maxmean_bwd_sums_kernel<float, float>), grid, dim3(1024), 0, S_(stream), (const float*)dy, arg, (const float*)H, (float*)dA, colsum, N, Tt, D);
+    else if (gdtype == 0) hipLaunchKernelGGL((maxmean_bwd_sums_kernel<bf16, float>), grid, dim3(1024), 0, S_(stream), (const float*)dy, arg, (const bf16*)H, (bf16*)dA, colsum, N, Tt, D);
+    else            hipLaunchKernelGGL((maxmean_bwd_sums_kernel<bf16, bf16>), grid, dim3(1024), 0, S_(stream), (const bf16*)dy, arg, (const bf16*)H, (bf16*)dA, colsum, N, Tt, D);
     ASSL_LAUNCH_CHECK();
 }
 
diff --git a/audio-ssl_amd/src/engine.py b/audio-ssl_amd/src/engine.py
--- a/audio-ssl_amd/src/engine.py
+++ b/audio-ssl_amd/src/engine.py
@@ -266,6 +266,8 @@
 LOSS_REPLICAS = 32
 _BN_STATS_P = os.environ.get("AUDIOSSL_BN_STATS_P", "1") != "0"
 _DP1_BF16 = os.environ.get("AUDIOSSL_DP1_BF16", "1") != "0"
+_DGRAD_BNSUMS = os.environ.get("AUDIOSSL_DGRAD_BNSUMS", "1") != "0"
+MAXMEAN_SUMS = os.environ.get("AUDIOSSL_MAXMEAN_SUMS", "1") != "0"
 
 
 def _conv_block_fwd(dtype, Pin, Nimg, Ti, Fi, W, bias, bn, train, update_running, col, packed=None):
@@ -419,14 +421,17 @@
     return x1, x2, x3, c.H2.view(Nimg, T3, d), c
 
 
-def _conv_block_bwd(dtype, Y, dP, dxl, st, Nimg, Ti, Fi, Pin, Wd, G_w, G_gamma, G_beta, need_dx, col, keep, dx_bf16=False, Pout=None):
+def _conv_block_bwd(dtype, Y, dP, dxl, st, Nimg, Ti, Fi, Pin, Wd, G_w, G_gamma, G_beta, need_dx, col, keep, dx_bf16=False, Pout=None,
+                    sums_in=None, sums_out=None):
     td = N.torch_dtype(dtype)
     scale, shift, mean, rstd = st
     M = Nimg * Ti * Fi
     dY = torch.empty((M, 64), dtype=td, device=Y.device)
-    stat = ARENA.scratch((33 * 128,), torch.float32, Y)
+    stat = sums_in if sums_in is not None else ARENA.scratch((33 * 128,), torch.float32, Y)
     yd = N.F32 if Y.dtype == torch.float32 else dtype
-    if SYNC_BN is None and Pout is not None and _BN_STATS_P and Pout.dtype == td:
+    if sums_in is not None:
+        N.call("bn_relu_pool_bwd_apply_sums", dtype, yd, GD, Y, dP, dxl, scale, shift, mean, rstd, stat, dY, G_gamma, G_beta, Nimg, Ti, Fi)
+    elif SYNC_BN is None and Pout is not None and _BN_STATS_P and Pout.dtype == td:
         N.call("bn_relu_pool_bwd_p", dtype, yd, GD, Y, Pout, dP, dxl, scale, shift, mean, rstd, stat, dY, G_gamma, G_beta, Nimg, Ti, Fi)
     elif SYNC_BN is None:
         N.call("bn_relu_pool_bwd", dtype, yd, GD, Y, dP, dxl, scale, shift, mean, rstd, stat, dY, G_gamma, G_beta, Nimg, Ti, Fi)
@@ -453,7 +458,10 @@
         return None
     dx_bf16 = dx_bf16 and fused
     dPin = _empty((Nimg, Ti, Fi, 64), torch.bfloat16 if dx_bf16 else torch.float32, like=Y)
-    if fused:
+    if fused and sums_out is not None:
+        dxl_in, st_in, stat_in = sums_out
+        N.call("conv3x3_dgrad_bnsums", dY, Wd, dPin, Pin, dxl_in, st_in[0], st_in[1], st_in[2], st_in[3], stat_in, Nimg, Ti, Fi)
+    elif fused:
         N.call("conv3x3_fwd", dY, Wd, None, dPin, 0 if dx_bf16 else 1, None, None, 1, Nimg, Ti, Fi)
     else:
         N.call("im2col3x3", dtype, dY, col, Nimg, Ti, Fi)
@@ -461,7 +469,7 @@
     return dPin
 
 
-def encoder_backward(c, G, dA2=None, dH2=None, dx1=None, dx2=None, dx3=None, dx_late=None, grads_zero=False):
+def encoder_backward(c, G, dA2=None, dH2=None, dx1=None, dx2=None, dx3=None, dx_late=None, grads_zero=False, dA2_colsum=None):
     dtype, Nimg, M, d, kin = c.dtype, c.N, c.M, c.d, c.kin
     T1, F1, T2, F2, T3, F3 = c.dims
     td = N.torch_dtype(dtype)
@@ -472,7 +480,10 @@
     dev = c.H2.device
     def w2():
         linear_bwd_w(dtype, dA2, c.H1, G["fc.3.weight"], M, d, d, dw_zero=grads_zero)
-        colsum_add(dtype, dA2, M, d, G["fc.3.bias"])
+        if dA2_colsum is not None:
+            N.call("add_d2f", dA2_colsum, G["fc.3.bias"], d)
+        else:
+            colsum_add(dtype, dA2, M, d, G["fc.3.bias"])
     WGRAD.run(dev, w2)
     scale = 1.0 / (1.0 - c.p_drop) if c.keep is not None else 1.0
     dA1 = linear_bwd_x(dtype, dA2, c.fw2, M, d, d, alpha=scale, gate=c.H1)
@@ -485,11 +496,15 @@
         dx1, dx2, dx3 = dx_late()
     col = _col_buffer(dtype, Nimg, T1, F1, c.H2)
     keep = []
+    stat2 = None
+    if SYNC_BN is None and dtype == N.BF16 and F2 == 16 and _BN_STATS_P and _DGRAD_BNSUMS and c.P2.dtype == td:
+        stat2 = ARENA.scratch((33 * 128,), torch.float32, c.H2)
     dP2 = _conv_block_bwd(dtype, c.Y3, dP3, dx3, c.st3, Nimg, T2, F2, c.P2, c.W3d, G["features_3.0.weight"],
-                          G["features_3.1.weight"], G["features_3.1.bias"], True, col, keep, Pout=c.P3)
+                          G["features_3.1.weight"], G["features_3.1.bias"], True, col, keep, Pout=c.P3,
+                          sums_out=(dx2, c.st2, stat2) if stat2 is not None else None)
     dP1 = _conv_block_bwd(dtype, c.Y2, dP2, dx2, c.st2, Nimg, T1, F1, c.P1, c.W2d, G["features_2.0.weight"],
                           G["features_2.1.weight"], G["features_2.1.bias"], True, col, keep, dx_bf16=bool(c.stem_mfma) and _DP1_BF16,
-                          Pout=c.P2)
+                          Pout=c.P2, sums_in=stat2)
     gd1 = N.BF16 if dP1.dtype == torch.bfloat16 else GD
     acc = ARENA.scratch((32 * 64 * 11,), torch.float32, c.H2)
     P = c.P
@@ -516,9 +531,13 @@
     return y, arg
 
 
-def maxmean_backward(dtype, dy, arg, H2):
+def maxmean_backward(dtype, dy, arg, H2, colsum=False):
     Nimg, T3, d = H2.shape
     dA2 = _empty((Nimg * T3, d), N.torch_dtype(dtype), like=H2)
+    if colsum:
+        sums = ARENA.scratch((d,), torch.float64, H2)
+        N.call("maxmean_bwd_sums", dtype, GD, dy, arg, H2, dA2, sums, Nimg, T3, d)
+        return dA2, sums
     N.call("maxmean_bwd", dtype, GD, dy, arg, H2, dA2, Nimg, T3, d)
     return dA2
 
diff --git a/audio-ssl_amd/src/upstream/delores_m/upstream_expert.py b/audio-ssl_amd/src/upstream/delores_m/upstream_expert.py
--- a/audio-ssl_amd/src/upstream/delores_m/upstream_expert.py
+++ b/audio-ssl_amd/src/upstream/delores_m/upstream_expert.py
@@ -195,15 +195,18 @@
             shadow = self.queue_shadow(dt)
             dq, kn32 = E.moco_forward_backward(dt, q, k, self.queue, shadow, float(self.hparams.softmax_temperature),
                                                loss[0:1], backward=need_grad)
-            dA2 = None
+            dA2 = dA2_sums = None
             if need_grad:
                 Gq = G("encoder_q.")
                 E.linear_bwd_w(dt, dq, yq, Gq["fc.weight"], B, wq.shape[0], wq.shape[1])
                 E.colsum_add(dt, dq, B, wq.shape[0], Gq["fc.bias"])
                 dyq = E.linear_bwd_x(dt, dq, wq, B, wq.shape[0], wq.shape[1], out_f32=1)
-                dA2 = E.maxmean_backward(dt, dyq, argq, Hq)
-            return kn32, dA2
-        kn32, dA2 = R.phase("moco", moco_phase)
+                if E.MAXMEAN_SUMS:
+                    dA2, dA2_sums = E.maxmean_backward(dt, dyq, argq, Hq, colsum=True)
+                else:
+                    dA2 = E.maxmean_backward(dt, dyq, argq, Hq)
+            return kn32, dA2, dA2_sums
+        kn32, dA2, dA2_sums = R.phase("moco", moco_phase)
         self._dequeue_and_enqueue(kn32, self.queue_shadow(dt) if dt != N.F32 else None)
         early_box = [None]
 
@@ -247,10 +250,10 @@
                         d = join_heads()
                         box[0] = loss.sum()
                         return d
-                    E.encoder_backward(cq, G("encoder_q.encoder."), dA2=dA2, dx_late=join_and_sum, grads_zero=_GRADS_ZERO)
+                    E.encoder_backward(cq, G("encoder_q.encoder."), dA2=dA2, dx_late=join_and_sum, grads_zero=_GRADS_ZERO, dA2_colsum=dA2_sums)
                     return box[0]
                 E.encoder_backward(cq, G("encoder_q.encoder."), dA2=dA2, dx1=dys[0], dx2=dys[1], dx3=dys[2],
-                                   grads_zero=_GRADS_ZERO)
+                                   grads_zero=_GRADS_ZERO, dA2_colsum=dA2_sums)
                 return loss.sum()
             total = R.phase("encoder_bwd", backward_phase)
             if early_box[0] is not None and not E.ONE_STREAM and _SGD_ASIDE:
diff --git a/include/audiossl_hip.h b/include/audiossl_hip.h
--- a/include/audiossl_hip.h
+++ b/include/audiossl_hip.h
@@ -84,6 +84,9 @@
 int audiossl_bn_relu_pool_bwd_p(int dtype, int ydtype, int gdtype, const void* Y, const void* P, const void* dP, const void* dxl,
                                 const float* scale, const float* shift, const float* mean, const float* rstd, float* stat, void* dY,
                                 float* dgamma, float* dbeta, int N, int Ti, int Fi, void* stream);
+int audiossl_bn_relu_pool_bwd_apply_sums(int dtype, int ydtype, int gdtype, const void* Y, const void* dP, const void* dxl,
+                                         const float* scale, const float* shift, const float* mean, const float* rstd, float* stat,
+                                         void* dY, float* dgamma, float* dbeta, int N, int Ti, int Fi, void* stream);
 int audiossl_conv1_moments(const float* img, int N, int F, int T, double* mom, void* stream);
 int audiossl_conv1_finalize(double* mom_totals, const float* w, const float* bias, const float* gamma, const float* beta,
                             float* running_mean, float* running_var, float momentum, float eps, double count, float* scale,
@@ -116,6 +119,9 @@
                          double* sumsq, int stat_replicas, int N, int Ti, int Fi, void* stream);
 int audiossl_conv3x3_wgrad(const void* dY, const void* X, float* dWp, float* workspace, long workspace_floats, int N, int Ti,
                            int Fi, void* stream);
+int audiossl_conv3x3_dgrad_bnsums(const void* dY, const void* W, void* dP, const void* P, const float* dxl, const float* scale,
+                                  const float* shift, const float* mean, const float* rstd, float* stat, int N, int Ti, int Fi,
+                                  void* stream);
 
 int audiossl_gemm(int dtype, int trans_a, int trans_b, int M, int N, int K, float alpha, const void* A, long lda,
                   const void* B, long ldb, void* C, long ldc, const float* bias, int relu, const uint8_t* keep, long ldk,
@@ -140,6 +146,8 @@
 int audiossl_maxmean_fwd(int dtype, int out_f32, const void* H, void* y, uint8_t* arg, int N, int Tt, int D, void* stream);
 int audiossl_maxmean_bwd(int dtype, int gdtype, const void* dy, const uint8_t* arg, const void* H, void* dA, int N, int Tt,
                          int D, void* stream);
+int audiossl_maxmean_bwd_sums(int dtype, int gdtype, const void* dy, const uint8_t* arg, const void* H, void* dA, double* colsum,
+                              int N, int Tt, int D, void* stream);
 
 int audiossl_colbn_fwd(int dtype, int adtype, const void* a, const float* scale, const float* shift, int relu, void* h,
                        int groups, long M, int C, void* stream);
```
